# skmhrk1209/GANSynth

Measured on AMD Instinct MI355X. Metric: G+D step images/sec at 128x1024x2 mel+IF, higher is better.
Workload: dtype bf16; 1 GPU; BASELINE.json configs[1]: fully grown PGGAN 128x1024x2 G+D iteration (D update + G update, R1 + mode-seeking), per-GPU batch 8, random-init weights; global_batch=8, parallelism=dp1, launch=hipGraph replay, forked branches, forked_branches=True

## Files before the change

### gansynth_amd/_lib.py

```python
import ctypes
import os
from ctypes import c_char_p, c_double, c_float, c_int, c_int64, c_size_t, c_void_p, POINTER

_HERE = os.path.dirname(os.path.abspath(__file__))
LIB_PATH = os.path.join(_HERE, "libgansynth_hip.so")

GS_F32, GS_BF16 = 0, 1
ACT_NONE, ACT_LRELU, ACT_TANH = 0, 1, 2
ACT_LRELU_BITS, ACT_WRITE_BITS = 5, 16
PREP_CONV_FWD, PREP_CONV_BWD_DATA, PREP_CONVT_FWD, PREP_CONVT_BWD_DATA = 0, 1, 2, 3
CONV_FWD, CONV_BWD_DATA, CONV_BWD_WEIGHT = 0, 1, 2

P, I, F, L, Z = c_void_p, c_int, c_float, c_int64, c_size_t

SIGNATURES = {
    "gs_last_error": (c_char_p, []),
    "gs_version": (I, []),
    "gs_init": (I, []),
    "gs_streams_create": (I, [I, POINTER(P)]),
    "gs_streams_destroy": (I, [I, POINTER(P)]),
    "gs_prof_enable": (I, [I]),
    "gs_prof_collect": (I, [POINTER(c_int), POINTER(c_double), POINTER(c_double)]),
    "gs_prof_roofline": (I, [ctypes.c_double, ctypes.c_double, P, P, P]),
    "gs_prof_records": (I, [I, P, P, P, P, P]),
    "gs_comm_available": (I, []),
    "gs_comm_unique_id": (I, [P]),
    "gs_comm_init": (I, [POINTER(P), I, I, P]),
    "gs_comm_destroy": (I, [P]),
    "gs_comm_count": (I, [P, POINTER(I)]),
    "gs_allreduce_sum_f32": (I, [P, P, ctypes.c_int64, P]),
    "gs_comm_set_marker_us": (I, [P, ctypes.c_double]),
    "gs_broadcast_f32": (I, [P, P, ctypes.c_int64, I, P]),
    "gs_conv2d_workspace_bytes": (Z, [I, I, I, I, I, I, I, I, I]),
    "gs_conv2d_fwd": (I, [P, P, P, I, I, I, I, I, I, I, F, I, I, P, Z, P]),
    "gs_conv2d_fwd_bias_act": (I, [P, P, P, P, I, I, I, I, I, I, I, F, I, I, I, P, Z, P]),
    "gs_conv2d_bwd_data": (I, [P, P, P, I, I, I, I, I, I, I, F, I, I, P, Z, P]),
    "gs_conv2d_fwd_bias_act_norm": (I, [P, P, P, P, P, I, I, I, I, I, I, I, F, I, F, I, I, P, Z, P]),
    "gs_conv2d_transpose_s2_fwd_bias_act_norm": (I, [P, P, P, P, P, I, I, I, I, I, F, I, F, I, I, P, Z, P]),
    "gs_conv2d_fwd_mask": (I, [P, P, P, I, P, I, I, I, I, I, I, I, F, I, I, P, Z, P]),
    "gs_conv2d_bwd_data_mask": (I, [P, P, P, I, P, I, I, I, I, I, I, I, F, I, I, P, Z, P]),
    "gs_conv2d_bwd_weight": (I, [P, P, P, I, I, I, I, I, I, I, F, I, I, P, Z, P]),
    "gs_conv2d_bwd_weight_bias": (I, [P, P, P, P, I, I, I, I, I, I, I, F, I, I, P, Z, P]),
    "gs_conv2d_bwd_weight_bias_partial": (I, [P, P, P, P, I, I, I, I, I, I, I, F, I, I, P, Z, P, P]),
    "gs_conv2d_transpose_s2_bwd_weight_partial": (I, [P, P, P, I, I, I, I, I, F, I, I, P, Z, P, P]),
    "gs_wgrad_reduce_batch": (I, [P, I, P]),
    "gs_conv2d_bwd_weight_bias_multi": (I, [P, P, P, I, ctypes.c_uint, P, P, I, I, I, I, I, I, I, F, I, I, P, Z, P, P]),
    "gs_conv2d_transpose_s2_bwd_weight_multi": (I, [P, P, P, I, P, I, I, I, I, I, F, I, I, P, Z, P, P]),
    "gs_conv_wgrad_jobs_workspace_bytes": (Z, [P, I]),
    "gs_conv_wgrad_jobs": (I, [P, I, P, Z, P]),
    "gs_wgrad_cu_cap": (I, [I]),
    "gs_conv2d_transpose_s2_workspace_bytes": (Z, [I, I, I, I, I, I, I]),
    "gs_conv2d_transpose_s2_fwd": (I, [P, P, P, I, I, I, I, I, F, I, I, P, Z, P]),
    "gs_conv2d_transpose_s2_fwd_bias_act": (I, [P, P, P, P, I, I, I, I, I, F, I, I, I, P, Z, P]),
    "gs_conv2d_transpose_s2_bwd_data": (I, [P, P, P, I, I, I, I, I, F, I, I, P, Z, P]),
    "gs_conv2d_bwd_data_pnbwd_is_fused": (I, [I, I, I, I, I, I, I, I, I]),
    "gs_conv2d_fwd_pnbwdbwd_is_fused": (I, [I, I, I, I, I, I, I, I, I]),
    "gs_conv_igemm_config": (I, [I, I, I, I, I, I, I, I, POINTER(c_int)]),
    "gs_units_bias_act_to_nhwc": (I, [P, P, P, P, I, I, I, I, I, P]),
    "gs_nhwc_act_bwd_to_units": (I, [P, P, P, I, I, I, I, I, P]),
    "gs_conv2d_fwd_pnbwdbwd": (I, [P, P, P, P, I, F, P, P, I, I, I, I, I, I, I, F, I, I, P, Z, P]),
    "gs_conv2d_transpose_s2_fwd_pnbwdbwd": (I, [P, P, P, P, I, F, P, P, I, I, I, I, I, F, I, I, P, Z, P]),
    "gs_conv2d_bwd_data_pnbwd": (I, [P, P, P, P, I, F, P, I, I, I, I, I, I, I, F, I, I, P, Z, P]),
    "gs_conv2d_transpose_s2_bwd_data_pnbwd": (I, [P, P, P, P, I, F, P, I, I, I, I, I, F, I, I, P, Z, P]),
    "gs_conv2d_transpose_s2_bwd_weight": (I, [P, P, P, I, I, I, I, I, F, I, I, P, Z, P]),
    "gs_dense_fwd_workspace_bytes": (Z, [I, I, I]),
    "gs_dense_fwd": (I, [P, P, P, I, I, I, F, I, P, Z, P]),
    "gs_dense_fwd_bias_act": (I, [P, P, P, P, I, I, I, F, I, I, P, Z, P]),
    "gs_dense_fwd_bias_act_nhwc": (I, [P, P, P, P, I, I, I, I, F, I, I, P, Z, P]),
    "gs_dense_bwd_data": (I, [P, P, P, I, I, I, F, I, P]),
    "gs_dense_bwd_weight": (I, [P, P, P, I, I, I, F, I, I, P]),
    "gs_dense_fwd_nhwc": (I, [P, P, P, I, I, I, I, F, I, P, Z, P]),
    "gs_dense_bwd_data_nhwc": (I, [P, P, P, I, I, I, I, F, I, P]),
    "gs_dense_bwd_weight_nhwc": (I, [P, P, P, I, I, I, I, F, I, I, P]),
    "gs_embedding_fwd": (I, [P, P, P, I, I, I, F, I, P]),
    "gs_embedding_onehot_fwd": (I, [P, P, P, P, I, I, I, F, I, P]),
    "gs_embedding_bwd": (I, [P, P, P, I, I, I, F, I, P]),
    "gs_bias_act_fwd": (I, [P, P, P, L, I, I, I, P]),
    "gs_act_bwd": (I, [P, P, P, L, I, I, P]),
    "gs_act_bwd_bias": (I, [P, P, P, P, L, I, I, I, I, P, Z, P]),
    "gs_tanh_bwd_bwd": (I, [P, P, P, P, L, I, P]),
    "gs_channel_sum_workspace_bytes": (Z, [L, I]),
    "gs_channel_sum": (I, [P, P, L, I, I, I, P, Z, P]),
    "gs_bias_partial_rows": (I, [I, L, I, I]),
    "gs_channel_fold_batch_workspace_bytes": (Z, [P, I]),
    "gs_channel_fold_batch": (I, [P, I, P, Z, P]),
    "gs_pixel_norm_fwd": (I, [P, P, L, I, F, I, P]),
    "gs_pixel_norm_bwd": (I, [P, P, P, L, I, F, I, P]),
    "gs_pixel_norm_bwd_fused": (I, [P, P, P, P, L, I, F, I, I, I, P]),
    "gs_pixel_norm_bwd_bias_workspace_bytes": (Z, [L, I, I]),
    "gs_pixel_norm_bwd_fused_bias": (I, [P, P, P, P, P, L, I, F, I, I, I, I, P, Z, P]),
    "gs_pixel_norm_bwd_bwd_fused": (I, [P, P, P, P, P, L, I, F, I, I, P]),
# ... 92 lines not shown
```

### gansynth_amd/config.py

```python
import os

KNOBS = {
    "GS_TORCH_COLLECTIVES": ("operational", "gradient all-reduce through torch.distributed's communicator instead of the library's own (gs_comm_*)"),
    "GS_NO_GRAPH_ALLREDUCE": ("operational", "no RCCL collective inside captured graphs: eager all-reduce behind each replay (bench.DP_LADDER's tamer modes)"),
    "GS_FORK_PROBE": ("operational", "auto | always | never: probe a forked hipGraph replay in a child process before the first forked capture "
                                     "(auto: only on HIP builds the workaround was not debugged on, fork_probe._forked_replay_ok)"),
    "GS_FORK_PROBED": ("operational", "(set by the probe for child processes: ok | died)"),
    "GS_FORK_PROBE_TIMEOUT_S": ("operational", "budget of that probe, seconds (600)"),
    "GS_LEVEL_STREAMS": ("operational", "throw-away streams alive while a graph is instantiated (128; capture.Capture._leveled_queues)"),
    "GS_COMM_MARKER_US": ("operational", "tests / profiles at world size 1: the one-rank all-reduce becomes a kernel that holds its stream this long "
                                         "(read once per communicator, comm.RcclComm; gs_comm_set_marker_us)"),
    "GS_CAPTURE_MODE": ("operational", "debugging: force torch.cuda.graph's capture_error_mode"),
    "GS_DEBUG_POISON_WS": ("operational", "debugging: kernel workspaces start as NaN bit patterns"),
    "GS_CHECK_FUSION": ("operational", "debugging: every fused cross-node form also runs its unfused definition and the two are compared"),
    "GS_FORK_EAGER": ("operational", "tests: the forked branches with eager launches on two streams"),
    "GS_NO_FORK_MARKS": ("operational", "debugging: branches start where they are opened, not at their marks"),
    "GS_NO_FORK": ("schedule", "no parallel branches in the runs' graphs (5.9 against 5.2 ms; also taken when GPU_MAX_HW_QUEUES != 4 or the probe fails)"),
    "GS_NO_MERGED_RUNS": ("schedule", "part A of the generator run NOT inside the discriminator run's graph (5.13 against 4.99 ms)"),
    "GS_NO_FUSED_ITERATION": ("schedule", "two graphs per iteration with eager optimizer steps between them (neutral on one GPU; data parallel both "
                                          "all-reduces are then the last node of a graph)"),
    "GS_OVERLAP_REDUCE": ("schedule", "data parallel: round 4's four-graph iteration, each all-reduce on a forked branch beside part A of the other run "
                                      "(hides both collectives; +0.7 ms at world size 1)"),
    "GS_NO_OVERLAP_REDUCE": ("schedule", "(overrides GS_OVERLAP_REDUCE)"),
    "GS_DEBUG_DP_BUCKET": ("operational", "print the range the first message of a two-step discriminator all-reduce covers"),
    "GS_DP_BUCKET_D": ("schedule", "data parallel: the discriminator's gradient all-reduced in two steps, ~98 % of it beside the end of its backward (300-us stand-ins: -0.09 ... -0.14 ms fully grown, +0.15 in a fade-in)"),
    "GS_EARLY_FLUSH_DIV": ("schedule", "a layer is 'large' from 1/DIV of the full resolution's pixels (16)"),
    "GS_EARLY_FLUSH_CUS": ("schedule", "CUs the early weight-gradient contraction is sized for (192; 160 / 224 / 256 within noise, round 6)"),
    "GS_D_TAIL_LEVELS": ("schedule", "levels of the discriminator's tail run over [real; fake] as one batch when the runs do not fork (3)"),
    "GS_NO_EARLY_FLUSH": ("ablation", "weight gradients of the full-chip levels contracted at the end of the run only"),
    "GS_NO_DEFERRED_REDUCE": ("ablation", "every weight gradient contracted where autograd produces it"),
    "GS_NO_DEFERRED_FOLDS": ("ablation", "bias-gradient partial rows folded by their producers"),
    "GS_NO_WGRAD_GROUPS": ("ablation", "no grouped weight-gradient launches"),
    "GS_NO_SPLIT_G_LOSS": ("ablation", "the generator's loss as one launch over both halves: the mode-seeking second-order pass waits for the discriminator's forward"),
    "GS_NO_SPLIT_FINAL_FLUSH": ("ablation", "the final weight-gradient contraction of a run on one stream (HBM-bound and MFMA-bound jobs one after the other)"),
    "GS_NO_FUSED_LOSSES": ("ablation", "per-sample loss algebra in torch instead of the one-launch loss heads"),
    "GS_NO_D_TAIL_BATCH": ("ablation", "real and fake pass through the discriminator's tail separately (no-fork schedule)"),
    "GS_NO_FUSED_NORM": ("ablation", "pixel norm as its own node behind every generator conv"),
    "GS_NO_NORM_EPILOGUE": ("ablation", "no pixel norm in conv epilogues"),
    "GS_NO_NORM_BWD_EPILOGUE": ("ablation", "no previous-block norm backward in data-gradient epilogues"),
    "GS_NO_NORM_BWD2_EPILOGUE": ("ablation", "no second-order norm kernel in the forward-on-cotangent conv"),
    "GS_NO_NORM_BWD_BIAS": ("ablation", "bias sums outside the norm's backward"),
    "GS_NO_MASK_BITS": ("ablation", "leaky-relu masks read as the bf16 activations themselves, not as the sign bits stored behind them"),
    "GS_NO_PREMASK": ("ablation", "activation derivative never folded into the consuming data-gradient kernel"),
    "GS_NO_PREMASK_GRAPH": ("ablation", "... not across autograd nodes"),
    "GS_NO_PREMASK_GRAPH2": ("ablation", "... not in second-order graphs"),
    "GS_NO_PARAMS_ONLY": ("ablation", "leaf activations receive gradients like tf.gradients would not ask for"),
    "GS_NO_DERIVED_SLICES": ("ablation", "the 257-channel conv's weight slices copied on every use"),
    "GS_NO_UNITS_NHWC": ("ablation", "dense -> reshape -> activation as three steps"),
    "GS_NO_DENSE_NHWC": ("ablation", "flatten copy + plain dense kernels"),
}


def _check(name):
    if name not in KNOBS:
        raise KeyError("gansynth_amd.config: %s is not a registered environment switch (add it to KNOBS with its description)" % name)


def flag(name):
    _check(name)
    return bool(os.environ.get(name))


def value(name, default=None):
    _check(name)
    return os.environ.get(name, default)
```

### gansynth_amd/csrc/conv_api.hip

```cpp
#include "conv_shared.h"
#include <utility>
#include <vector>

namespace gs {


bool igemm_supported(int ic, int oc, int dtype);
bool igemm_norm_fused(int mode, int N, int Hb, int Wb, int IC, int OC, int dtype, int want);
int igemm_config(int mode, int N, int Hb, int Wb, int IC, int OC, int dtype, int want, int* out);
extern "C" int gs_pixel_norm_bwd_bwd_fused(const void* gg, const void* g, const void* x, void* out, void* out_g, int64_t p, int c, float eps, int pre_act,
                                           int dtype, void* stream);
bool wgrad_mfma_supported(int ic, int oc, int dtype);
size_t igemm_prep_bytes(int ic, int oc, int dtype);
int run_igemm(int mode, int variant, const void* x, const float* w_hwio, void* y, int N, int Hi, int Wi, int ICk,
              int OCk, int w_ci, int w_co, int Hb, int Wb, float alpha, const float* bias, int act, int dtype, int w_prepared,
              void* ws, size_t ws_bytes, hipStream_t st, const void* mask = nullptr, int mask_act = 0, void* y2 = nullptr, float pn_eps = 0.f,
              const void* addend = nullptr, int normbwd = 0);
extern "C" int gs_pixel_norm_bwd_fused(const void* g, const void* x, const void* addend, void* gx, int64_t p, int c, float eps, int pre_act, int post_act, int dtype,
                                       void* stream);
size_t wgrad_mfma_bytes(int mode, int dtype, int N, int Hb, int Wb, int IC, int OC);
bool wgrad_mfma_has_bias(int dtype);
int run_wgrad_mfma(int mode, const WgradSrcs& srcs, int nsrc, float* gw, float* gb, int N, int Hi, int Wi, int IC, int OC, int Hb,
                   int Wb, float alpha, int transpose, int accumulate, int dtype, void* ws, size_t ws_bytes, hipStream_t st,
                   GsWgradReduce* defer = nullptr);
bool wgrad_sk_supported(int mode, int dtype, int IC, int OC);
int wgrad_sk_tile_width(int Wb);
void wgrad_sk_job_geometry(int mode, int tw, int N, SkJob& q);
void wgrad_sk_plan(int mode, SkGroup& g);
size_t wgrad_sk_bytes(const SkGroup& g);
int run_wgrad_sk(int mode, int tw, const SkGroup& g, void* ws, size_t ws_bytes, hipStream_t st);

template <typename T, int OCV, int VEC>
__global__ void conv_direct_kernel(const T* __restrict__ x, const float* __restrict__ wp, T* __restrict__ y, int mode,
                                   int ks, int N, int Hi, int Wi, int IC, int OC, int Ho, int Wo, float alpha) {
    const int ngrp = OC / OCV;
    const long idx = (long)blockIdx.x * blockDim.x + threadIdx.x;
    const long total = (long)N * Ho * Wo * ngrp;
    if (idx >= total) return;
    const int g = idx % ngrp;
    long pix = idx / ngrp;
    const int ox = pix % Wo;
    pix /= Wo;
    const int oy = pix % Ho;
    const int n = pix / Ho;
    const int oc = g * OCV;
    float acc[OCV];
#pragma unroll
    for (int v = 0; v < OCV; ++v) acc[v] = 0.f;
    for (int ky = 0; ky < ks; ++ky) {
        int iy;
        if (mode == MODE_S1) iy = oy + ky - (ks >> 1);
        else if (mode == MODE_S2) iy = 2 * oy + ky;
        else { const int d = oy - ky; if (d < 0 || (d & 1)) continue; iy = d >> 1; }
        if (iy < 0 || iy >= Hi) continue;
        for (int kx = 0; kx < ks; ++kx) {
            int ix;
            if (mode == MODE_S1) ix = ox + kx - (ks >> 1);
            else if (mode == MODE_S2) ix = 2 * ox + kx;
            else { const int d = ox - kx; if (d < 0 || (d & 1)) continue; ix = d >> 1; }
            if (ix < 0 || ix >= Wi) continue;
            const T* xp = x + (((long)n * Hi + iy) * Wi + ix) * IC;
            const float* wr = wp + ((long)(ky * ks + kx) * OC + oc) * IC;
            if (VEC == 4) {
                for (int ic = 0; ic < IC; ic += 4) {
                    float xv[4];
                    ld4(xp + ic, xv);
#pragma unroll
                    for (int v = 0; v < OCV; ++v) {
                        const float4 wv = *reinterpret_cast<const float4*>(wr + (long)v * IC + ic);
                        acc[v] += xv[0] * wv.x + xv[1] * wv.y + xv[2] * wv.z + xv[3] * wv.w;
// ... 773 lines not shown
    if (int e = run_direct(mode, ksize, 0, x, w_hwio, z, n, h, w, ci, co, ci, co, hb, wb, alpha, dtype, w_prepared, ws, ws_bytes, st, bias, act, &fused, nullptr, 0, nullptr,
                           bits_out, &bits_done))
        return e;
    if (!fused && (bias || act != GS_ACT_NONE))
        if (int e = gs_bias_act_fwd(z, bias, z, (int64_t)n * hb * wb, co, act, dtype, stream)) return e;
    if (y2)
        if (int e = gs_pixel_norm_fwd(z, y2, (int64_t)n * hb * wb, co, pn_eps, dtype, stream)) return e;
    if (want_bits && !bits_done) return gs_pack_act_bits(y, (int64_t)n * hb * wb, co, dtype, stream);
    return 0;
}

extern "C" int gs_conv2d_fwd(const void* x, const float* w_hwio, void* y, int n, int h, int w, int ci, int co, int ksize,
                             int stride, float alpha, int dtype, int w_prepared, void* ws, size_t ws_bytes, void* stream) {
    return conv2d_fwd_impl(x, w_hwio, nullptr, GS_ACT_NONE, y, n, h, w, ci, co, ksize, stride, alpha, dtype, w_prepared, ws, ws_bytes, stream);
}

extern "C" int gs_conv2d_fwd_bias_act(const void* x, const float* w_hwio, const float* bias, void* y, int n, int h, int w, int ci, int co,
                                      int ksize, int stride, float alpha, int act, int dtype, int w_prepared, void* ws, size_t ws_bytes,
                                      void* stream) {
    return conv2d_fwd_impl(x, w_hwio, bias, act, y, n, h, w, ci, co, ksize, stride, alpha, dtype, w_prepared, ws, ws_bytes, stream);
}

extern "C" int gs_act_bwd(const void* g, const void* y, void* gx, int64_t numel, int act, int dtype, void* stream);

extern "C" int gs_conv2d_fwd_mask(const void* x, const float* w_hwio, const void* mask, int mask_act, void* y, int n, int h, int w, int ci, int co,
                                  int ksize, int stride, float alpha, int dtype, int w_prepared, void* ws, size_t ws_bytes, void* stream) {
    if (int e = check_conv_args(n, h, w, ci, co, ksize, stride, dtype)) return e;
    GS_CHECK_ARG(mask == nullptr || mask_act == GS_ACT_LRELU || mask_act == GS_ACT_TANH || mask_act == GS_ACT_LRELU_BITS, "conv2d_fwd_mask: bad activation %d", mask_act);
    hipStream_t st = as_stream(stream);
    const int hb = h / stride, wb = w / stride;
    const int mode = stride == 2 ? MODE_S2 : MODE_S1;
    const bool fused = mask != nullptr && co >= mask_fuse_min_channels() && ksize == 3 && igemm_supported(ci, co, dtype);
    int rc;
    const int bits_act = mask_act;
    if (mask_act == GS_ACT_LRELU_BITS) mask_act = GS_ACT_LRELU;
    if (ksize == 3 && igemm_supported(ci, co, dtype))
        rc = run_igemm(mode, 0, x, w_hwio, y, n, h, w, ci, co, ci, co, hb, wb, alpha, nullptr, GS_ACT_NONE, dtype, w_prepared, ws, ws_bytes, st, fused ? mask : nullptr, bits_act);
    else {
        bool epi = false, mdone = false;
        rc = run_direct(mode, ksize, 0, x, w_hwio, y, n, h, w, ci, co, ci, co, hb, wb, alpha, dtype, w_prepared, ws, ws_bytes, st, nullptr, GS_ACT_NONE, &epi, mask, mask_act, &mdone);
        if (rc || !mask || mdone) return rc;
    }
    if (rc || !mask || fused) return rc;
    return gs_act_bwd(y, mask, y, (int64_t)n * hb * wb * co, mask_act, dtype, stream);
}

extern "C" int gs_conv2d_fwd_bias_act_norm(const void* x, const float* w_hwio, const float* bias, void* z, void* y, int n, int h, int w, int ci, int co,
                                           int ksize, int stride, float alpha, int act, float eps, int dtype, int w_prepared, void* ws,
                                           size_t ws_bytes, void* stream) {
    GS_CHECK_ARG(y != nullptr, "conv2d_fwd_bias_act_norm: y is required (z is optional)");
    return conv2d_fwd_impl(x, w_hwio, bias, act, z, n, h, w, ci, co, ksize, stride, alpha, dtype, w_prepared, ws, ws_bytes, stream, y, eps);
}

extern "C" int gs_act_bwd(const void* g, const void* y, void* gx, int64_t numel, int act, int dtype, void* stream);

extern "C" int gs_conv2d_bwd_data_mask(const void* gy, const float* w_hwio, const void* mask, int mask_act, void* gx, int n, int h, int w, int ci, int co,
                                       int ksize, int stride, float alpha, int dtype, int w_prepared, void* ws, size_t ws_bytes, void* stream) {
    if (int e = check_conv_args(n, h, w, ci, co, ksize, stride, dtype)) return e;
    GS_CHECK_ARG(mask == nullptr || mask_act == GS_ACT_LRELU || mask_act == GS_ACT_TANH || mask_act == GS_ACT_LRELU_BITS, "conv2d_bwd_data_mask: bad activation %d", mask_act);
    const int bits_act = mask_act;
    if (mask_act == GS_ACT_LRELU_BITS) mask_act = GS_ACT_LRELU;
    const float* bias = nullptr;
    const int act = GS_ACT_NONE;
    hipStream_t st = as_stream(stream);
    const int hb = h / stride, wb = w / stride;
    int rc;
    bool fused = mask != nullptr && ci >= mask_fuse_min_channels();
    const void* km = fused ? mask : nullptr;
    if (stride == 1) {
        if (ksize == 3 && igemm_supported(co, ci, dtype))
            rc = run_igemm(MODE_S1, 1, gy, w_hwio, gx, n, h, w, co, ci, ci, co, h, w, alpha, bias, act, dtype, w_prepared, ws, ws_bytes, st, km, bits_act);
        else { rc = run_direct(MODE_S1, ksize, 1, gy, w_hwio, gx, n, h, w, co, ci, ci, co, h, w, alpha, dtype, w_prepared, ws, ws_bytes, st); fused = false; }
    } else if (igemm_supported(co, ci, dtype)) {
        rc = run_igemm(MODE_T2, 2, gy, w_hwio, gx, n, hb, wb, co, ci, ci, co, hb, wb, alpha, bias, act, dtype, w_prepared, ws, ws_bytes, st, km, bits_act);
    } else {
        rc = run_direct(MODE_T2, 3, 2, gy, w_hwio, gx, n, hb, wb, co, ci, ci, co, h, w, alpha, dtype, w_prepared, ws, ws_bytes, st);
        fused = false;
    }
    if (rc || !mask || fused) return rc;
    return gs_act_bwd(gx, mask, gx, (int64_t)n * h * w * ci, mask_act, dtype, stream);
}

extern "C" int gs_conv2d_bwd_data(const void* gy, const float* w_hwio, void* gx, int n, int h, int w, int ci, int co,
                                  int ksize, int stride, float alpha, int dtype, int w_prepared, void* ws, size_t ws_bytes, void* stream) {
    return gs_conv2d_bwd_data_mask(gy, w_hwio, nullptr, 0, gx, n, h, w, ci, co, ksize, stride, alpha, dtype, w_prepared, ws, ws_bytes, stream);
}

extern "C" size_t gs_channel_sum_workspace_bytes(int64_t p, int c);
extern "C" int gs_channel_sum(const void* g, float* out, int64_t p, int c, int accumulate, int dtype, void* ws, size_t ws_bytes, void* stream);

static WgradSrcs make_srcs(const void* const* xs, const void* const* gys, int nsrc, int n_per, const int* ns, unsigned bias_mask, bool swap, int* total) {
    WgradSrcs s;
    memset(&s, 0, sizeof(s));
    int end = 0;
    for (int i = 0; i < GS_WGRAD_MAX_SRC; ++i) {
        if (i < nsrc) {
            s.x[i] = swap ? gys[i] : xs[i];
            s.gy[i] = swap ? xs[i] : gys[i];
            end += ns ? ns[i] : n_per;
        }
        s.n_end[i] = end;
    }
    s.bias_mask = bias_mask;
    *total = end;
    return s;
}
// ... 197 lines not shown
                                                 jb.accumulate, jb.dtype, jws, jbytes, &d, stream);
        if (rc) return rc;
        if (jb.gw_ci_stride > jb.ci) {
            if (d.nslices <= 0 || d.transpose) return fail(GS_ERR_UNSUPPORTED, "conv_wgrad_jobs: a %d -> %d layer cannot add into a channel slice", jb.ci, jb.co);
            d.ic_ld = jb.gw_ci_stride;
        }
        if (d.nslices > 0) pend.push_back(d);
    }
    if (!pend.empty()) return gs_wgrad_reduce_batch(pend.data(), (int)pend.size(), stream);
    return 0;
}

extern "C" int gs_conv2d_bwd_weight(const void* x, const void* gy, float* gw_hwio, int n, int h, int w, int ci, int co,
                                    int ksize, int stride, float alpha, int accumulate, int dtype, void* ws, size_t ws_bytes, void* stream) {
    return gs_conv2d_bwd_weight_bias(x, gy, gw_hwio, nullptr, n, h, w, ci, co, ksize, stride, alpha, accumulate, dtype, ws, ws_bytes, stream);
}

extern "C" size_t gs_conv2d_transpose_s2_workspace_bytes(int which, int n, int h, int w, int ci, int co, int dtype) {
    if (which == GS_CONV_BWD_WEIGHT) {
        if (wgrad_mfma_supported(co, ci, dtype)) return wgrad_mfma_bytes(MODE_S2, dtype, n, h, w, co, ci);
        return wgrad_direct_bytes(3, n, h, w, co, ci);
    }
    return align256((size_t)9 * ci * co * 4);
}

static int conv2d_transpose_fwd_impl(const void* x, const float* w_hwio, const float* bias, int act, void* y, int n, int h, int w, int ci,
                                     int co, float alpha, int dtype, int w_prepared, void* ws, size_t ws_bytes, void* stream, void* y2 = nullptr,
                                     float pn_eps = 0.f) {
    if (int e = check_conv_args(n, 2 * h, 2 * w, co, ci, 3, 2, dtype)) return e;
    GS_CHECK_ARG(y || y2, "conv2d_transpose: no output");
    hipStream_t st = as_stream(stream);
    if (igemm_supported(ci, co, dtype) && act != GS_ACT_TANH)
        return run_igemm(MODE_T2, 0, x, w_hwio, y, n, h, w, ci, co, ci, co, h, w, alpha, bias, act, dtype, w_prepared, ws, ws_bytes, st, nullptr, 0, y2, pn_eps);
    void* z = y ? y : y2;
    if (int e = run_direct(MODE_T2, 3, 0, x, w_hwio, z, n, h, w, ci, co, ci, co, 2 * h, 2 * w, alpha, dtype, w_prepared, ws, ws_bytes, st)) return e;
    if (bias || act != GS_ACT_NONE)
        if (int e = gs_bias_act_fwd(z, bias, z, (int64_t)n * 4 * h * w, co, act, dtype, stream)) return e;
    if (y2) return gs_pixel_norm_fwd(z, y2, (int64_t)n * 4 * h * w, co, pn_eps, dtype, stream);
    return 0;
}

extern "C" int gs_conv2d_transpose_s2_fwd(const void* x, const float* w_hwio, void* y, int n, int h, int w, int ci, int co,
                                          float alpha, int dtype, int w_prepared, void* ws, size_t ws_bytes, void* stream) {
    return conv2d_transpose_fwd_impl(x, w_hwio, nullptr, GS_ACT_NONE, y, n, h, w, ci, co, alpha, dtype, w_prepared, ws, ws_bytes, stream);
}

extern "C" int gs_conv2d_transpose_s2_fwd_bias_act_norm(const void* x, const float* w_hwio, const float* bias, void* z, void* y, int n, int h, int w,
                                                        int ci, int co, float alpha, int act, float eps, int dtype, int w_prepared, void* ws,
                                                        size_t ws_bytes, void* stream) {
    GS_CHECK_ARG(y != nullptr, "conv2d_transpose_s2_fwd_bias_act_norm: y is required (z is optional)");
    return conv2d_transpose_fwd_impl(x, w_hwio, bias, act, z, n, h, w, ci, co, alpha, dtype, w_prepared, ws, ws_bytes, stream, y, eps);
}

extern "C" int gs_conv2d_transpose_s2_fwd_bias_act(const void* x, const float* w_hwio, const float* bias, void* y, int n, int h, int w, int ci,
                                                   int co, float alpha, int act, int dtype, int w_prepared, void* ws, size_t ws_bytes,
                                                   void* stream) {
    return conv2d_transpose_fwd_impl(x, w_hwio, bias, act, y, n, h, w, ci, co, alpha, dtype, w_prepared, ws, ws_bytes, stream);
}

extern "C" int gs_conv2d_transpose_s2_bwd_data(const void* gy, const float* w_hwio, void* gx, int n, int h, int w, int ci,
                                               int co, float alpha, int dtype, int w_prepared, void* ws, size_t ws_bytes, void* stream) {
    if (int e = check_conv_args(n, 2 * h, 2 * w, co, ci, 3, 2, dtype)) return e;
    const float* bias = nullptr;
    const int act = GS_ACT_NONE;
    hipStream_t st = as_stream(stream);
    if (igemm_supported(co, ci, dtype))
        return run_igemm(MODE_S2, 2, gy, w_hwio, gx, n, 2 * h, 2 * w, co, ci, ci, co, h, w, alpha, bias, act, dtype, w_prepared, ws, ws_bytes, st);
    return run_direct(MODE_S2, 3, 2, gy, w_hwio, gx, n, 2 * h, 2 * w, co, ci, ci, co, h, w, alpha, dtype, w_prepared, ws, ws_bytes, st);
}

extern "C" int gs_conv2d_fwd_pnbwdbwd(const void* x, const float* w_hwio, const void* g, const void* z, int act, float eps, void* out_g, void* out_z, int n, int h,
                                      int w, int ci, int co, int ksize, int stride, float alpha, int dtype, int w_prepared, void* ws, size_t ws_bytes, void* stream) {
    if (int e = check_conv_args(n, h, w, ci, co, ksize, stride, dtype)) return e;
    GS_CHECK_ARG(g && z && out_g && out_z && (act == GS_ACT_NONE || act == GS_ACT_LRELU), "conv2d_fwd_pnbwdbwd: g, z and both outputs are required, activation none or leaky relu (got %d)", act);
    hipStream_t st = as_stream(stream);
    const int hb = h / stride, wb = w / stride;
    if (ksize == 3 && igemm_supported(ci, co, dtype))
        return run_igemm(stride == 2 ? MODE_S2 : MODE_S1, 0, x, w_hwio, out_g, n, h, w, ci, co, ci, co, hb, wb, alpha, nullptr, GS_ACT_NONE, dtype, w_prepared, ws, ws_bytes, st,
                         z, act, out_z, eps, g, 2);
    if (int e = gs_conv2d_fwd(x, w_hwio, out_g, n, h, w, ci, co, ksize, stride, alpha, dtype, w_prepared, ws, ws_bytes, stream)) return e;
    return gs_pixel_norm_bwd_bwd_fused(out_g, g, z, out_z, out_g, (int64_t)n * hb * wb, co, eps, act, dtype, stream);
}
extern "C" int gs_conv2d_transpose_s2_fwd_pnbwdbwd(const void* x, const float* w_hwio, const void* g, const void* z, int act, float eps, void* out_g, void* out_z, int n,
                                                   int h, int w, int ci, int co, float alpha, int dtype, int w_prepared, void* ws, size_t ws_bytes, void* stream) {
    if (int e = check_conv_args(n, 2 * h, 2 * w, co, ci, 3, 2, dtype)) return e;
    GS_CHECK_ARG(g && z && out_g && out_z && (act == GS_ACT_NONE || act == GS_ACT_LRELU), "conv2d_transpose_s2_fwd_pnbwdbwd: g, z and both outputs are required, activation none or leaky relu (got %d)", act);
    hipStream_t st = as_stream(stream);
    if (igemm_supported(ci, co, dtype))
        return run_igemm(MODE_T2, 0, x, w_hwio, out_g, n, h, w, ci, co, ci, co, h, w, alpha, nullptr, GS_ACT_NONE, dtype, w_prepared, ws, ws_bytes, st, z, act, out_z, eps, g, 2);
    if (int e = gs_conv2d_transpose_s2_fwd(x, w_hwio, out_g, n, h, w, ci, co, alpha, dtype, w_prepared, ws, ws_bytes, stream)) return e;
    return gs_pixel_norm_bwd_bwd_fused(out_g, g, z, out_z, out_g, (int64_t)n * 4 * h * w, co, eps, act, dtype, stream);
}
extern "C" int gs_conv2d_fwd_pnbwdbwd_is_fused(int n, int h, int w, int ci, int co, int ksize, int stride, int transposed, int dtype) {
    if (ksize != 3 || !igemm_supported(ci, co, dtype)) return 0;
    if (transposed) return stride == 2 && igemm_norm_fused(MODE_T2, n, h, w, ci, co, dtype, IGEMM_NORM_BWD2) ? 1 : 0;
    return stride == 1 && igemm_norm_fused(MODE_S1, n, h, w, ci, co, dtype, IGEMM_NORM_BWD2) ? 1 : 0;
}

extern "C" int gs_conv2d_bwd_data_pnbwd(const void* gy, const float* w_hwio, const void* z, const void* addend, int act, float eps, void* gx, int n, int h, int w,
                                        int ci, int co, int ksize, int stride, float alpha, int dtype, int w_prepared, void* ws, size_t ws_bytes, void* stream) {
    if (int e = check_conv_args(n, h, w, ci, co, ksize, stride, dtype)) return e;
    GS_CHECK_ARG(z && gx && (act == GS_ACT_NONE || act == GS_ACT_LRELU), "conv2d_bwd_data_pnbwd: z is required, activation none or leaky relu (got %d)", act);
    hipStream_t st = as_stream(stream);
    if (stride == 1 && ksize == 3 && igemm_supported(co, ci, dtype))
        return run_igemm(MODE_S1, 1, gy, w_hwio, gx, n, h, w, co, ci, ci, co, h, w, alpha, nullptr, GS_ACT_NONE, dtype, w_prepared, ws, ws_bytes, st, z, act, nullptr, eps, addend, 1);
    if (stride == 1 && thin_expand_pnbwd_ok(ksize, co, ci, dtype)) {
// ... 64 lines not shown
```

### gansynth_amd/csrc/conv_igemm.hip

```cpp
#include <type_traits>
#include "conv_shared.h"
#include "gs_prof.h"

#ifndef GS_WGRAD_THIN_PREFETCH
#define GS_WGRAD_THIN_PREFETCH 1
#endif

extern "C" int gs_pixel_norm_fwd(const void* x, void* y, int64_t p, int c, float eps, int dtype, void* stream);
extern "C" int gs_pack_act_bits(void* z, int64_t p, int c, int dtype, void* stream);
extern "C" int gs_pixel_norm_bwd_fused(const void* g, const void* x, const void* addend, void* gx, int64_t p, int c, float eps, int pre_act, int post_act, int dtype,
                                       void* stream);
extern "C" int gs_pixel_norm_bwd_bwd_fused(const void* gg, const void* g, const void* x, void* out, void* out_g, int64_t p, int c, float eps, int pre_act,
                                           int dtype, void* stream);

namespace gs {

typedef float f32x16 __attribute__((ext_vector_type(16)));
typedef float f32x4 __attribute__((ext_vector_type(4)));
typedef __bf16 bf16x8 __attribute__((ext_vector_type(8)));


template <typename T> struct Mma;
template <> struct Mma<float> {
    typedef f32x4 frag_t;
    __device__ static inline void mma(const frag_t& a, const frag_t& b, f32x16& c) {
        c = __builtin_amdgcn_mfma_f32_32x32x2f32(a[0], b[0], c, 0, 0, 0);
        c = __builtin_amdgcn_mfma_f32_32x32x2f32(a[1], b[1], c, 0, 0, 0);
        c = __builtin_amdgcn_mfma_f32_32x32x2f32(a[2], b[2], c, 0, 0, 0);
        c = __builtin_amdgcn_mfma_f32_32x32x2f32(a[3], b[3], c, 0, 0, 0);
    }
};
template <> struct Mma<bf16_t> {
    typedef bf16x8 frag_t;
    __device__ static inline void mma(const frag_t& a, const frag_t& b, f32x16& c) {
        c = __builtin_amdgcn_mfma_f32_32x32x16_bf16(a, b, c, 0, 0, 0);
    }
};

template <int MODE> __host__ __device__ constexpr int patch_dim(int t) {
    return MODE == MODE_S1 ? t + 2 : (MODE == MODE_S2 ? 2 * t + 1 : t + 1);
}
template <int MODE> __host__ __device__ constexpr int tap_ky(int i) {
    return MODE == MODE_T2 ? (i < 4 ? (i >> 1) * 2 : (i < 6 ? (i - 4) * 2 : 1)) : i / 3;
}
template <int MODE> __host__ __device__ constexpr int tap_kx(int i) {
    return MODE == MODE_T2 ? (i < 4 ? (i & 1) * 2 : (i < 6 ? 1 : (i < 8 ? (i - 6) * 2 : 1))) : i % 3;
}
template <int MODE> __host__ __device__ constexpr int tap_phase(int i) {
    return MODE == MODE_T2 ? (i < 4 ? 0 : (i < 6 ? 1 : (i < 8 ? 2 : 3))) : 0;
}
template <int MODE> __host__ __device__ constexpr int tap_off(int k) {
    return MODE == MODE_T2 ? (k == 2 ? 0 : 1) : k;
}

struct ConvP {
    const void* x;
    const void* wp;
    void* y;
    const float* bias;
    int act;
    const void* mask;
    int mask_act;
    const unsigned char* mask_bits;
    unsigned char* bits_out;
    void* y2;
    float pn_eps;
    const void* addend;
    int normbwd;
    int* norm_pending;
    int N, Hi, Wi, IC, OC, Hb, Wb, tiles_x, tiles_y, nsp, noct, nch;
    unsigned m_noct, m_tx, m_ty;
    float alpha;
#ifdef GS_IGEMM_TRACE
    unsigned long long* trace;
#endif
};
#ifdef GS_IGEMM_TRACE
#define GS_TR(slot)                                                                                              \
    do {                                                                                                         \
        if (p.trace && threadIdx.x == 0 && (slot) < 64) {                                                        \
            p.trace[blockIdx.x * 64 + (slot)] = __builtin_amdgcn_s_memtime();                                    \
            if ((slot) == 0 || (slot) == 63) p.trace[4096 * 64 + blockIdx.x * 2 + ((slot) == 63)] = __builtin_amdgcn_s_memrealtime(); \
        }                                                                                                        \
    } while (0)
#else
#define GS_TR(slot) do { } while (0)
#endif

template <int N, int I = 0, typename F>
__device__ __forceinline__ void static_for(F&& f) {
    if constexpr (I < N) {
        f(std::integral_constant<int, I>{});
        static_for<N, I + 1>(f);
    }
}

typedef int i32x4 __attribute__((ext_vector_type(4)));

__device__ __forceinline__ void lds_dma16(unsigned lds_addr, unsigned voff, i32x4 rs) {
    asm volatile("s_mov_b32 m0, %0\n\ts_nop 0\n\tbuffer_load_dwordx4 %1, %2, 0 offen lds"
                 :
                 : "s"(lds_addr), "v"(voff), "s"(rs)
                 : "memory", "m0");
}
__device__ __forceinline__ void lds_dma16_s(unsigned lds_addr, unsigned voff, i32x4 rs, unsigned soff) {
    asm volatile("s_mov_b32 m0, %0\n\ts_nop 0\n\tbuffer_load_dwordx4 %1, %2, %3 offen lds"
                 :
                 : "s"(lds_addr), "v"(voff), "s"(rs), "s"(__builtin_amdgcn_readfirstlane(soff))
                 : "memory", "m0");
}
#ifndef GS_THIN_DMA_NT
#define GS_THIN_DMA_NT 0
#endif
__device__ __forceinline__ void lds_dma16_stream(unsigned lds_addr, unsigned voff, i32x4 rs) {
#if GS_THIN_DMA_NT
    asm volatile("s_mov_b32 m0, %0\n\ts_nop 0\n\tbuffer_load_dwordx4 %1, %2, 0 offen nt lds"
                 :
                 : "s"(lds_addr), "v"(voff), "s"(rs)
                 : "memory", "m0");
#else
    lds_dma16(lds_addr, voff, rs);
#endif
}
__device__ __forceinline__ i32x4 make_rsrc(const void* base, unsigned bytes) {
    const unsigned long long b = reinterpret_cast<unsigned long long>(base);
// ... 6 lines not shown
}
__device__ __forceinline__ void wait_vmcnt(int n) {
#define GS_VM(K) case K: asm volatile("s_waitcnt vmcnt(" #K ")" ::: "memory"); break;
    switch (n) {
        GS_VM(0) GS_VM(1) GS_VM(2) GS_VM(3) GS_VM(4) GS_VM(5) GS_VM(6) GS_VM(7) GS_VM(8) GS_VM(9) GS_VM(10) GS_VM(11)
        GS_VM(12) GS_VM(13) GS_VM(14) GS_VM(15) GS_VM(16) GS_VM(17) GS_VM(18) GS_VM(19) GS_VM(20) GS_VM(21) GS_VM(22)
        GS_VM(23) GS_VM(24) GS_VM(25) GS_VM(26) GS_VM(27) GS_VM(28) GS_VM(29) GS_VM(30) GS_VM(31) GS_VM(32)
        default: asm volatile("s_waitcnt vmcnt(0)" ::: "memory"); break;
    }
#undef GS_VM
}
__device__ __forceinline__ void block_barrier() {
    asm volatile("s_waitcnt lgkmcnt(0)" ::: "memory");
    __builtin_amdgcn_s_barrier();
    asm volatile("" ::: "memory");
}

#ifndef GS_NORM_EPI_PIPELINE
#define GS_NORM_EPI_PIPELINE 1
#endif
template <typename T, int MODE, int A, int B, int TW, int TG, bool RESIDENT, int D, int NORM, int RB = 64, bool SPEC = false, bool BITS = false>
__global__ __launch_bounds__(SPEC ? 512 : 256) void conv_igemm_kernel(const ConvP p) {
    static_assert(NORM >= 0 && NORM <= 3, "NORM: 0 plain, 1 pixel norm of the result (forward blocks), 2 pixel-norm backward of the result (data gradients), "
                                          "3 both gradients of a differentiated norm backward (second-order pass)");
    constexpr int NP = 128 * B;
    constexpr int TH = NP / TW;
    constexpr int PH = patch_dim<MODE>(TH), PW = patch_dim<MODE>(TW);
    constexpr int S = MODE == MODE_S2 ? 2 : 1;
    constexpr int NPH = MODE == MODE_T2 ? 4 : 1;
    constexpr int SZ = (int)sizeof(T);
    static_assert(RB == 64 || (RB == 128 && SZ == 2), "128-byte rows: bf16 only");
    constexpr int BK = RB / SZ;
    constexpr int SL = RB / 16;
    constexpr int KS = RB / 32;
    constexpr int OCT = 32 * A;
    constexpr int NTG = 9 / TG;
    constexpr int PCH = PH * PW * SL;
    constexpr int NPP = (PCH + 63) / 64;
    constexpr int PP = (NPP + 3) / 4;
    constexpr int PBUF = PP * 4096;
    constexpr int WBYTES = TG * OCT * RB;
    constexpr int NWP = WBYTES / 1024;
    constexpr int WP = (NWP + 3) / 4;
    constexpr int WBUF = WP * 4096;
    constexpr int NPB = 1 + (D + NTG - 1) / NTG;
    constexpr int NWB = D + 1;
    constexpr int NSTEP = KS * TG;
    typedef typename Mma<T>::frag_t frag_t;

    extern __shared__ __attribute__((aligned(16))) unsigned char lds[];
    unsigned char* const lpatch = lds;
    unsigned char* const lwgt = lds + NPB * PBUF;
    float* const lbias = reinterpret_cast<float*>(lwgt + (RESIDENT ? p.nch : NWB) * WBUF);
    const unsigned a_patch = (unsigned)(uintptr_t)lds;
    const unsigned a_wgt = a_patch + NPB * PBUF;

    const T* __restrict__ wp = reinterpret_cast<const T*>(p.wp);
    T* __restrict__ y = reinterpret_cast<T*>(p.y);
    const int Hi = p.Hi, Wi = p.Wi, IC = p.IC, OC = p.OC, Hb = p.Hb, Wb = p.Wb, NCH = p.nch;

    const int tid = threadIdx.x;
    const int lane = tid & 63, hi = lane >> 5, l31 = lane & 31;
    const int wv8 = __builtin_amdgcn_readfirstlane(tid >> 6);
    const bool loader = SPEC && wv8 >= 4;
    const bool issuer = !SPEC || loader;
    const bool computer = !SPEC || !loader;
    const int wv = wv8 & 3;

    const int total = p.nsp * p.noct;
    int first, stride, count;
    if ((gridDim.x & 7) == 0) {
        const int per_xcd = (total + 7) >> 3, gx = gridDim.x >> 3;
        const int xcd = blockIdx.x & 7, loc = blockIdx.x >> 3;
        first = xcd * per_xcd + loc;
        stride = gx;
        int end = (xcd + 1) * per_xcd;
        if (end > total) end = total;
        count = first < end ? (end - first + gx - 1) / gx : 0;
    } else {
        first = blockIdx.x;
        stride = gridDim.x;
        count = first < total ? (total - first + stride - 1) / stride : 0;
    }
    if (count == 0) return;
    GS_TR(0);

    int p_voff[PP], p_lx[PP];
#pragma unroll
    for (int k = 0; k < PP; ++k) {
        const int slot = (wv + 4 * k) * 64 + lane;
        const int row = slot / SL, pos = slot % SL;
        const int ly = row / PW, lx = row - ly * PW;
        p_voff[k] = ((ly * Wi + lx) * IC) * SZ + ((pos ^ (RB == 64 ? (lx >> 2) & 3 : (lx >> 1) & 7)) << 4);
        p_lx[k] = slot < PCH ? lx : 0x40000000;
    }
    constexpr int RPP = 1024 / RB;
    constexpr int SUBS = OCT / RPP;
    const int w_lane0 = RB == 64 ? ((lane >> 2) * IC) * SZ + (((lane & 3) ^ ((lane >> 4) & 3)) << 4)
                                 : ((lane >> 3) * IC) * SZ + (((lane & 7) ^ (lane >> 4)) << 4);
    const int w_lane1 = RB == 64 ? w_lane0 : ((lane >> 3) * IC) * SZ + (((lane & 7) ^ (4 + (lane >> 4))) << 4);
    int w_soff[NTG][WP];
    bool w_odd[WP];
#pragma unroll
    for (int k = 0; k < WP; ++k) w_odd[k] = RB == 128 && (((wv + 4 * k) % SUBS) & 1);
#pragma unroll
    for (int tg = 0; tg < NTG; ++tg)
// ... 65 lines not shown
                --i_left;
                i_item += stride;
                if (i_left > 0) item_coords(i_item, i_n, i_by, i_bx, i_oc0);
                else i_left = 0;
            }
        }
    };

    f32x16 acc[NPH][A][B];
    auto zero_acc = [&]() __attribute__((always_inline)) {
#pragma unroll
        for (int ph = 0; ph < NPH; ++ph)
#pragma unroll
            for (int a = 0; a < A; ++a)
#pragma unroll
                for (int b = 0; b < B; ++b)
#pragma unroll
                    for (int r = 0; r < 16; ++r) acc[ph][a][b][r] = 0.f;
    };

    int b_off[B][3][KS], a_off[KS];
#pragma unroll
    for (int b = 0; b < B; ++b) {
        const int q = (wv * B + b) * 32 + l31;
        const int pb0 = ((q / TW) * S) * PW + (q % TW) * S;
#pragma unroll
        for (int ox = 0; ox < 3; ++ox) {
            const int lx = (q % TW) * S + ox;
            const int key = RB == 64 ? (lx >> 2) & 3 : (lx >> 1) & 7;
#pragma unroll
            for (int ks = 0; ks < KS; ++ks) b_off[b][ox][ks] = (pb0 + ox) * RB + (((ks * 2 + hi) ^ key) << 4);
        }
    }
#pragma unroll
    for (int ks = 0; ks < KS; ++ks) a_off[ks] = l31 * RB + (((ks * 2 + hi) ^ (RB == 64 ? (l31 >> 2) & 3 : (l31 >> 1) & 7)) << 4);

    GS_TR(1);
    if (issuer) {
        if (RESIDENT) {
            for (int ch = 0; ch < NCH; ++ch)
#pragma unroll
                for (int k = 0; k < WP; ++k) issue_weight_piece(k, 0, (i_oc0 * IC + ch * BK) * SZ, a_wgt + ch * WBUF);
        }
#pragma unroll
        for (int d = 0; d < D; ++d) {
            issue_setup(d % NTG);
#pragma unroll
            for (int q = 0; q < stage_pieces(d % NTG); ++q) issue_piece(q, d % NTG);
            issue_advance(d % NTG);
        }
    }
    GS_TR(2);
    for (int c = tid; c < OC; c += (SPEC ? 512 : 256)) lbias[c] = p.bias ? p.bias[c] : 0.f;
    zero_acc();
    if (computer) {
#pragma unroll
        for (int b = 0; b < B; ++b)
#pragma unroll
            for (int ox = 0; ox < 3; ++ox)
#pragma unroll
                for (int ks = 0; ks < KS; ++ks) asm volatile("" : "+v"(b_off[b][ox][ks]));
#pragma unroll
        for (int ks = 0; ks < KS; ++ks) asm volatile("" : "+v"(a_off[ks]));
#pragma unroll
        for (int ph = 0; ph < NPH; ++ph)
#pragma unroll
            for (int a = 0; a < A; ++a)
#pragma unroll
                for (int b = 0; b < B; ++b) asm volatile("" : "+v"(acc[ph][a][b]));
    }
    wait_vmcnt(0);
    block_barrier();
    GS_TR(3);
#ifdef GS_IGEMM_TRACE
    int tr_stage = 0;
#endif

    int item = first, done = 0, c_pb = 0, c_wb = 0;
    while (true) {
        int n, by, bx, oc0;
        item_coords(item, n, by, bx, oc0);
        unsigned mbw[BITS ? B * (MODE == MODE_T2 ? 4 : 1) : 1][A];
        constexpr bool NPIPE = (NORM == 2 || NORM == 3) && A * B <= 2 && GS_NORM_EPI_PIPELINE;
        typedef typename std::conditional<SZ == 4, float4, uint4>::type nvec_t;
        constexpr int NNV = SZ == 4 ? 4 : 2;
        nvec_t nz[NPIPE ? 2 : 1][A][NNV], nx[NPIPE ? 2 : 1][A][NNV];
        auto norm_fetch = [&](int i, nvec_t (&zq)[A][NNV], nvec_t (&xq)[A][NNV]) __attribute__((always_inline)) {
            constexpr int NPHB = MODE == MODE_T2 ? 4 : 1;
            const int b = i / NPHB, ph = i % NPHB;
            const int Ho = MODE == MODE_T2 ? 2 * Hb : Hb, Wo = MODE == MODE_T2 ? 2 * Wb : Wb;
            const int q = (wv * B + b) * 32 + l31;
            const int gy = by + q / TW, gx = bx + q % TW;
            const int oy = MODE == MODE_T2 ? 2 * gy + (ph >> 1) : gy;
            const int ox = MODE == MODE_T2 ? 2 * gx + (ph & 1) : gx;
            const long base = (gy < Hb && gx < Wb) ? (((long)n * Ho + oy) * Wo + ox) * OC + oc0 : 0;
#ifdef GS_ABL_NOMASKLOAD
            const long zbase = base & 1023;
#else
            const long zbase = base;
#endif
#pragma unroll
            for (int a = 0; a < A; ++a)
#pragma unroll
                for (int v = 0; v < NNV; ++v) {
                    zq[a][v] = *reinterpret_cast<const nvec_t*>(reinterpret_cast<const T*>(p.mask) + zbase + a * 32 + v * (32 / NNV) + hi * (16 / NNV));
                    if (NORM == 3 || p.addend)
// ... 369 lines not shown
                                        }
                                }
                                ssq = swap32_sum(ssq); shg = swap32_sum(shg);
                                shz = swap32_sum(shz); szg = swap32_sum(szg);
                                const float inv_c = 1.f / (float)(32 * A);
                                const float r = rsqrtf(ssq * inv_c + p.pn_eps);
                                const float r2 = r * r, r3 = r2 * r;
                                const float ma = shg * inv_c, mb = shz * inv_c, mm = szg * inv_c;
                                const float kz = 3.f * r3 * r2 * mb * mm - r3 * ma;
#pragma unroll
                                for (int a = 0; a < A; ++a)
#pragma unroll
                                    for (int v = 0; v < NV; ++v) {
                                        float o1[EV], o2[EV];
#pragma unroll
                                        for (int e = 0; e < EV; ++e) {
                                            const float zc = zv[a][v][e], gc = gv[a][v][e], hc = hv[a][v][e];
                                            o1[e] = r * (hc - zc * r2 * mb);
                                            o2[e] = kz * zc - r3 * (mm * hc + mb * gc);
                                        }
                                        if (inside) {
                                            if constexpr (SZ == 4) {
                                                st4(reinterpret_cast<float*>(y) + off + a * 32 + v * 8 + hi * 4, o1);
                                                st4(reinterpret_cast<float*>(p.y2) + off + a * 32 + v * 8 + hi * 4, o2);
                                            } else {
                                                uint4 w4;
                                                w4.x = pack_bf16x2(o1[0], o1[1]); w4.y = pack_bf16x2(o1[2], o1[3]); w4.z = pack_bf16x2(o1[4], o1[5]); w4.w = pack_bf16x2(o1[6], o1[7]);
                                                *reinterpret_cast<uint4*>(reinterpret_cast<bf16_t*>(y) + off + a * 32 + v * 16 + hi * 8) = w4;
                                                w4.x = pack_bf16x2(o2[0], o2[1]); w4.y = pack_bf16x2(o2[2], o2[3]); w4.z = pack_bf16x2(o2[4], o2[5]); w4.w = pack_bf16x2(o2[6], o2[7]);
                                                *reinterpret_cast<uint4*>(reinterpret_cast<bf16_t*>(p.y2) + off + a * 32 + v * 16 + hi * 8) = w4;
                                            }
                                        }
                                    }
                            } else if constexpr (NORM == 1) {
                                float o[A][4][4], ssq = 0.f;
#pragma unroll
                                for (int a = 0; a < A; ++a) {
                                    finish(ph, a, b, o[a]);
#pragma unroll
                                    for (int k = 0; k < 16; ++k) ssq += o[a][k >> 2][k & 3] * o[a][k >> 2][k & 3];
                                }
                                ssq = swap32_sum(ssq);
                                const float r = rsqrtf(ssq * (1.f / (float)(32 * A)) + p.pn_eps);
#pragma unroll
                                for (int a = 0; a < A; ++a) {
                                    if (y) {
                                        float oz[4][4];
#pragma unroll
                                        for (int k = 0; k < 16; ++k) oz[k >> 2][k & 3] = o[a][k >> 2][k & 3];
                                        store(y, off, a, oz, inside, static_cast<const mvec_t*>(nullptr));
                                    }
#pragma unroll
                                    for (int k = 0; k < 16; ++k) o[a][k >> 2][k & 3] *= r;
                                    store(reinterpret_cast<T*>(p.y2), off, a, o[a], inside, static_cast<const mvec_t*>(nullptr));
                                }
                            } else {
                                mvec_t mz_one[A][NV];
                                if constexpr (!MASK_ALL) {
                                    if (p.mask) mask_fetch(off, inside, mz_one);
                                }
#pragma unroll
                                for (int a = 0; a < A; ++a) {
                                    float o[4][4];
                                    finish(ph, a, b, o);
                                    const mvec_t* mz = MASK_ALL ? mz_all[MASK_ALL ? b * NPH + ph : 0][a] : mz_one[a];
                                    store(y, off, a, o, inside, mz, p.mask ? (use_mb ? 2 : 1) : 0, emit_bits);
                                }
                            }
                        }
                    }
                    zero_acc();
                }
#endif
                block_barrier();
#ifdef GS_IGEMM_TRACE
                GS_TR(4 + tr_stage);
                ++tr_stage;
#endif
                if (tg == NTG - 1) c_pb = c_pb + 1 == NPB ? 0 : c_pb + 1;
                if (!RESIDENT) c_wb = c_wb + 1 == NWB ? 0 : c_wb + 1;
            }
        }
        if (++done >= count) break;
        item += stride;
    }
    GS_TR(63);
    wait_vmcnt(0);
}

template <typename T, int MODE, int TW>
__global__ __launch_bounds__(256) void conv_wgrad_kernel(
    const WgradSrcs srcs, float* __restrict__ part,
    int N, int Hi, int Wi, int IC, int OC, int Hb, int Wb, int tiles_x, int tiles_y, int ntiles, int nslices) {
    constexpr int NP = MODE == MODE_S2 ? 64 : 128;
    constexpr int TH = NP / TW;
    constexpr int PH = patch_dim<MODE>(TH), PW = patch_dim<MODE>(TW);
    constexpr int S = MODE == MODE_S2 ? 2 : 1;
    constexpr int ROWF = 32;
    constexpr int LDS_MAIN = (PH * PW + NP) * ROWF;
    constexpr int LDS_RED = 4 * 1024;
    __shared__ __attribute__((aligned(16))) float lds[LDS_MAIN > LDS_RED ? LDS_MAIN : LDS_RED];
    float* lp = lds;
    float* lg = lds + PH * PW * ROWF;

    const int tid = threadIdx.x;
    const int lane = tid & 63, wv = tid >> 6, hi = lane >> 5, l31 = lane & 31;
    const int n_ict = IC / 32;
// ... 920 lines not shown
static int g_wgrad_cu_cap = 0;
static int wgrad_cus() {
    const int n = num_cus();
    return g_wgrad_cu_cap > 0 && g_wgrad_cu_cap < n ? g_wgrad_cu_cap : n;
}

#ifndef GS_MAX_BLOCKS_PER_CU
#define GS_MAX_BLOCKS_PER_CU 2
#endif
#ifndef GS_SMALL_D
#define GS_SMALL_D 2
#endif
template <typename T, int MODE, int A, int B, int TW, int TG, bool RESIDENT = false, int D = 2, int NORM = 0, int RB = 64, bool SPEC = false, bool BITS = false>
static int launch_igemm(ConvP p, hipStream_t st) {
    if constexpr (!BITS && sizeof(T) == 2 && NORM == 0) {
        if (p.mask_bits || p.bits_out) return launch_igemm<T, MODE, A, B, TW, TG, RESIDENT, D, NORM, RB, SPEC, true>(p, st);
    }
    constexpr int NP = 128 * B;
    constexpr int TH = NP / TW;
    constexpr int PH = patch_dim<MODE>(TH), PW = patch_dim<MODE>(TW);
    constexpr int OCT = 32 * A;
    constexpr int BK = RB / (int)sizeof(T);
    constexpr int NTG = 9 / TG;
    constexpr int PBUF = ((PH * PW * (RB / 16) + 255) / 256) * 4096;
    constexpr int WBUF = ((TG * OCT * RB + 4095) / 4096) * 4096;
    constexpr int NPB = 1 + (D + NTG - 1) / NTG, NWB = D + 1;
    p.tiles_x = cdiv(p.Wb, TW);
    p.tiles_y = cdiv(p.Hb, TH);
    p.nsp = p.N * p.tiles_x * p.tiles_y;
    p.noct = cdiv(p.OC, OCT);
    p.nch = p.IC / BK;
    {
        auto magic = [](int d) { return d <= 1 ? 0u : (unsigned)(((1ull << 32) + (unsigned)d - 1) / (unsigned)d); };
        if (p.noct >= 2048 || p.tiles_x >= 2048 || p.tiles_y >= 2048)
            return fail(GS_ERR_UNSUPPORTED, "conv igemm: %d channel tiles / %d x %d spatial tiles exceed the item decoder's range", p.noct, p.tiles_x, p.tiles_y);
        static const long max_items = getenv("GS_IGEMM_MAX_ITEMS") ? atol(getenv("GS_IGEMM_MAX_ITEMS")) : (1L << 21);
        if ((long)p.nsp * p.noct >= max_items) {
            const long per_image = (long)p.tiles_x * p.tiles_y * p.noct;
            const int chunk = (int)((max_items - 1) / per_image);
            if (chunk < 1) return fail(GS_ERR_UNSUPPORTED, "conv igemm: %ld work items per image exceed the item decoder's range", per_image);
            const size_t in_img = (size_t)p.Hi * p.Wi * p.IC * sizeof(T);
            const size_t out_img = (size_t)p.Hb * p.Wb * (MODE == MODE_T2 ? 4 : 1) * p.OC * sizeof(T);
            auto adv = [](const void* q, size_t b) -> const void* { return q ? (const char*)q + b : nullptr; };
            for (int n0 = 0; n0 < p.N; n0 += chunk) {
                ConvP q = p;
                q.N = p.N - n0 < chunk ? p.N - n0 : chunk;
                q.x = adv(p.x, n0 * in_img);
                q.y = const_cast<void*>(adv(p.y, n0 * out_img));
                q.y2 = const_cast<void*>(adv(p.y2, n0 * out_img));
                q.mask = adv(p.mask, n0 * out_img);
                q.mask_bits = reinterpret_cast<const unsigned char*>(adv(p.mask_bits, n0 * out_img / (8 * sizeof(T))));
                q.bits_out = reinterpret_cast<unsigned char*>(const_cast<void*>(adv(p.bits_out, n0 * out_img / (8 * sizeof(T)))));
                q.addend = adv(p.addend, n0 * out_img);
                int pending = 0;
                if (p.norm_pending) q.norm_pending = &pending;
                if (int e = launch_igemm<T, MODE, A, B, TW, TG, RESIDENT, D, NORM, RB, SPEC, BITS>(q, st)) return e;
                if (p.norm_pending && pending) *p.norm_pending = pending;
            }
            return 0;
        }
        p.m_noct = magic(p.noct); p.m_tx = magic(p.tiles_x); p.m_ty = magic(p.tiles_y);
    }
    const int wbufs = RESIDENT ? p.nch : NWB;
    const size_t lds = (size_t)NPB * PBUF + (size_t)wbufs * WBUF + (size_t)((p.OC + 3) / 4) * 16 + 0;
    if (p.OC % OCT != 0) return fail(GS_ERR_UNSUPPORTED, "conv igemm: %d output channels with %d-wide tiles", p.OC, OCT);
    if ((size_t)p.Hi * p.Wi * p.IC * sizeof(T) >= (1ull << 31)) return fail(GS_ERR_UNSUPPORTED, "conv igemm: one image exceeds 2 GiB");
    if (lds > 160 * 1024) return fail(GS_ERR_UNSUPPORTED, "conv igemm: %zu bytes of LDS needed", lds);
    if (NORM && p.OC != OCT) return fail(GS_ERR_UNSUPPORTED, "conv igemm: fused pixel norm needs the whole channel range in one tile");
    if ((NORM == 2 || NORM == 3) && p.OC != OCT) return fail(GS_ERR_UNSUPPORTED, "conv igemm: fused pixel-norm backward needs the whole channel range in one tile");
    if (!((NORM == 2 && p.normbwd == 1) || (NORM == 3 && p.normbwd == 2)) && p.normbwd) {
        if (p.norm_pending) *p.norm_pending = 1 + p.normbwd;
        p.normbwd = 0;
        p.mask = nullptr;
        p.addend = nullptr;
        p.y2 = nullptr;
    }
    if (NORM != 1 && NORM != 3 && p.y2) {
        if (!p.y) p.y = p.y2;
        p.y2 = nullptr;
        if (p.norm_pending) *p.norm_pending = 1;
    }
    if (p.IC % BK != 0) return fail(GS_ERR_UNSUPPORTED, "conv igemm: %d input channels with %d-channel chunks", p.IC, BK);
    auto kern = conv_igemm_kernel<T, MODE, A, B, TW, TG, RESIDENT, D, NORM, RB, SPEC, BITS>;
    static size_t max_set = 0;
    if (lds > max_set) {
        if (hipFuncSetAttribute(reinterpret_cast<const void*>(kern), hipFuncAttributeMaxDynamicSharedMemorySize, (int)lds) != hipSuccess)
            return fail(GS_ERR_HIP, "conv igemm: cannot reserve %zu bytes of dynamic LDS", lds);
        max_set = lds;
    }
    int per_cu = (int)((160 * 1024) / lds);
    if (per_cu > GS_MAX_BLOCKS_PER_CU) per_cu = GS_MAX_BLOCKS_PER_CU;
    if (per_cu < 1 || SPEC) per_cu = 1;
    const long total = (long)p.nsp * p.noct;
    long grid = (long)per_cu * num_cus();
    if (grid > total) grid = total;
    if (grid >= 8) grid &= ~7L;
    const double flops = 2.0 * 9.0 * (double)p.N * p.Hb * p.Wb * p.IC * p.OC;
    const double out_px = (double)p.N * p.Hb * p.Wb * (MODE == MODE_T2 ? 4 : 1);
    const double bytes = ((double)p.N * p.Hi * p.Wi * p.IC + out_px * p.OC * (1.0 + (p.mask ? (p.mask_bits ? 1.0 / 16.0 : 1.0) : 0.0) + (p.bits_out ? 1.0 / 16.0 : 0.0) + ((NORM == 1 && p.y) ? 1.0 : 0.0) + ((NORM == 2 && p.addend) ? 1.0 : 0.0) + (NORM == 3 ? 2.0 : 0.0)) + 9.0 * p.IC * p.OC) * sizeof(T);
    const int reps = prof_reps();
    ProfScope ps(st, flops, bytes, MODE, p.N, p.Hb, p.Wb, p.IC, p.OC, p.mask ? 1 : 0, NORM ? 1 : 0, reps);
    for (int r = 0; r < reps; ++r) hipLaunchKernelGGL(kern, dim3((unsigned)grid), dim3(SPEC ? 512 : 256), lds, st, p);
    return 0;
}

struct IgemmCfg {
    int A, B, TW, TG;
    bool RESIDENT = false;
    int D = 2, NORM = IGEMM_PLAIN, RB = 64;
    bool SPEC = false;
    bool operator==(const IgemmCfg& o) const {
        return A == o.A && B == o.B && TW == o.TW && TG == o.TG && RESIDENT == o.RESIDENT && D == o.D && NORM == o.NORM && RB == o.RB && SPEC == o.SPEC;
    }
};
struct IgemmKnobs { bool no_small_tiles, no_rb128, spec; };
static IgemmKnobs igemm_knobs() {
    static const IgemmKnobs k = {getenv("GS_NO_SMALL_TILES") != nullptr, getenv("GS_NO_RB128") != nullptr,
                                 getenv("GS_SPEC") ? (atoi(getenv("GS_SPEC")) & 1) != 0 : true};
    return k;
}

static IgemmCfg choose_igemm(int mode, int dtype, int N, int Hb, int Wb, int IC, int OC, int want, long cus, IgemmKnobs knobs) {
    constexpr int FWD = 1 << IGEMM_NORM_FWD, BWD = 1 << IGEMM_NORM_BWD, BWD2 = 1 << IGEMM_NORM_BWD2;
    auto epi = [&](int forms) { return (forms >> want) & 1 ? want : IGEMM_PLAIN; };
    const int nch = IC / (dtype == GS_F32 ? 16 : 32);
    const bool a2 = OC % 64 == 0;
    const int tw = Wb >= 32 ? 32 : 16;
    auto items64 = [&](int B_) { return (long)N * cdiv(Hb, 4 * B_) * cdiv(Wb, 32) * (OC / 64); };
    const bool small = !knobs.no_small_tiles && items64(1) <= cus;
    const bool rb128 = dtype == GS_BF16 && !knobs.no_rb128 && IC % 64 == 0;
    if (mode == MODE_S2) {
        if (small) return {1, 1, tw, 9, false, 1};
        if (!a2) return {1, 1, 32, 3};
        if (OC == 64 && nch == 1 && Wb >= 32 && items64(1) >= cus) return {2, 1, 32, 9, true, 1, epi(BWD)};
        if (OC % 128 == 0 && Wb >= 32 && (long)N * cdiv(Hb, 4) * cdiv(Wb, 32) * (OC / 128) >= cus) return {4, 1, 32, 3};
        return {2, 1, tw, 3};
    }
    const bool s1 = mode == MODE_S1;
    if (OC == 32 && nch <= 2 && Wb >= 64) return {1, s1 ? 2 : 1, 64, 9, true, 1, epi(s1 ? FWD | BWD | BWD2 : FWD | BWD2)};
    if (small) {
        if (rb128) return {1, 1, tw, 9, false, 1, IGEMM_PLAIN, 128, knobs.spec};
        return {1, 1, tw, 9, false, GS_SMALL_D};
    }
    if (!a2) return {1, 1, s1 ? 32 : tw, 3};
    if (!s1) return {2, 1, tw, 3, false, 2, Wb >= 32 && OC == 64 ? epi(FWD | BWD2) : IGEMM_PLAIN};
    if (Wb >= 32 && items64(2) >= 2 * cus) return {2, 2, 32, 3, false, 1, OC == 64 ? epi(FWD | BWD | BWD2) : IGEMM_PLAIN};
    if (OC == 64 && nch <= 2 && Wb >= 32 && items64(2) >= cus / 2) return {2, 2, 32, 9, true};
    if (Wb >= 32 && items64(2) >= cus) {
        if (rb128) return {2, 2, 32, 3, false, 1, IGEMM_PLAIN, 128};
        return {2, 2, 32, 3};
    }
    return {2, 1, tw, 3};
// ... 11 lines not shown
    X(MODE_S1, false, 1, 2, 64, 9, true, 1, IGEMM_NORM_BWD, 64, false)          \
    X(MODE_S1, false, 1, 2, 64, 9, true, 1, IGEMM_NORM_BWD2, 64, false)         \
    X(MODE_S1, true, 1, 1, 32, 9, false, 1, IGEMM_PLAIN, 128, true)             \
    X(MODE_S1, true, 1, 1, 16, 9, false, 1, IGEMM_PLAIN, 128, true)             \
    X(MODE_S1, true, 1, 1, 32, 9, false, 1, IGEMM_PLAIN, 128, false)            \
    X(MODE_S1, true, 1, 1, 16, 9, false, 1, IGEMM_PLAIN, 128, false)            \
    X(MODE_S1, false, 1, 1, 32, 9, false, GS_SMALL_D, IGEMM_PLAIN, 64, false)   \
    X(MODE_S1, false, 1, 1, 16, 9, false, GS_SMALL_D, IGEMM_PLAIN, 64, false)   \
    X(MODE_S1, false, 1, 1, 32, 3, false, 2, IGEMM_PLAIN, 64, false)            \
    X(MODE_S1, false, 2, 2, 32, 3, false, 1, IGEMM_PLAIN, 64, false)            \
    X(MODE_S1, false, 2, 2, 32, 3, false, 1, IGEMM_NORM_FWD, 64, false)         \
    X(MODE_S1, false, 2, 2, 32, 3, false, 1, IGEMM_NORM_BWD, 64, false)         \
    X(MODE_S1, false, 2, 2, 32, 3, false, 1, IGEMM_NORM_BWD2, 64, false)        \
    X(MODE_S1, false, 2, 2, 32, 9, true, 2, IGEMM_PLAIN, 64, false)             \
    X(MODE_S1, true, 2, 2, 32, 3, false, 1, IGEMM_PLAIN, 128, false)            \
    X(MODE_S1, false, 2, 2, 32, 3, false, 2, IGEMM_PLAIN, 64, false)            \
    X(MODE_S1, false, 2, 1, 32, 3, false, 2, IGEMM_PLAIN, 64, false)            \
    X(MODE_S1, false, 2, 1, 16, 3, false, 2, IGEMM_PLAIN, 64, false)            \
    X(MODE_S2, false, 1, 1, 32, 9, false, 1, IGEMM_PLAIN, 64, false)            \
    X(MODE_S2, false, 1, 1, 16, 9, false, 1, IGEMM_PLAIN, 64, false)            \
    X(MODE_S2, false, 1, 1, 32, 3, false, 2, IGEMM_PLAIN, 64, false)            \
    X(MODE_S2, false, 2, 1, 32, 9, true, 1, IGEMM_PLAIN, 64, false)             \
    X(MODE_S2, false, 2, 1, 32, 9, true, 1, IGEMM_NORM_BWD, 64, false)          \
    X(MODE_S2, false, 4, 1, 32, 3, false, 2, IGEMM_PLAIN, 64, false)            \
    X(MODE_S2, false, 2, 1, 32, 3, false, 2, IGEMM_PLAIN, 64, false)            \
    X(MODE_S2, false, 2, 1, 16, 3, false, 2, IGEMM_PLAIN, 64, false)            \
    X(MODE_T2, false, 1, 1, 64, 9, true, 1, IGEMM_PLAIN, 64, false)             \
    X(MODE_T2, false, 1, 1, 64, 9, true, 1, IGEMM_NORM_FWD, 64, false)          \
    X(MODE_T2, false, 1, 1, 64, 9, true, 1, IGEMM_NORM_BWD2, 64, false)         \
    X(MODE_T2, true, 1, 1, 32, 9, false, 1, IGEMM_PLAIN, 128, true)             \
    X(MODE_T2, true, 1, 1, 16, 9, false, 1, IGEMM_PLAIN, 128, true)             \
    X(MODE_T2, true, 1, 1, 32, 9, false, 1, IGEMM_PLAIN, 128, false)            \
    X(MODE_T2, true, 1, 1, 16, 9, false, 1, IGEMM_PLAIN, 128, false)            \
    X(MODE_T2, false, 1, 1, 32, 9, false, GS_SMALL_D, IGEMM_PLAIN, 64, false)   \
    X(MODE_T2, false, 1, 1, 16, 9, false, GS_SMALL_D, IGEMM_PLAIN, 64, false)   \
    X(MODE_T2, false, 1, 1, 32, 3, false, 2, IGEMM_PLAIN, 64, false)            \
    X(MODE_T2, false, 1, 1, 16, 3, false, 2, IGEMM_PLAIN, 64, false)            \
    X(MODE_T2, false, 2, 1, 32, 3, false, 2, IGEMM_PLAIN, 64, false)            \
    X(MODE_T2, false, 2, 1, 32, 3, false, 2, IGEMM_NORM_FWD, 64, false)         \
    X(MODE_T2, false, 2, 1, 32, 3, false, 2, IGEMM_NORM_BWD2, 64, false)        \
    X(MODE_T2, false, 2, 1, 16, 3, false, 2, IGEMM_PLAIN, 64, false)            \
    GS_IGEMM_FORCED(X)

static bool igemm_instantiated(int mode, int dtype, const IgemmCfg& c) {
#define GS_ROW(M, BF16_ONLY, ...) if (mode == M && (dtype == GS_BF16 || !BF16_ONLY) && c == IgemmCfg{__VA_ARGS__}) return true;
    GS_IGEMM_CONFIGS(GS_ROW)
#undef GS_ROW
    return false;
}

template <typename T, int MODE>
static int dispatch_igemm(ConvP p, hipStream_t st) {
    constexpr int dtype = sizeof(T) == 4 ? GS_F32 : GS_BF16;
    const int want = p.normbwd ? 1 + p.normbwd : (p.y2 ? IGEMM_NORM_FWD : IGEMM_PLAIN);
    IgemmCfg c = choose_igemm(MODE, dtype, p.N, p.Hb, p.Wb, p.IC, p.OC, want, num_cus(), igemm_knobs());
#ifdef GS_FORCE_CFG
    if (MODE == GS_FORCE_MODE && dtype == GS_BF16) c = IgemmCfg{GS_FORCE_CFG};
#endif
#define GS_ROW(M, BF16_ONLY, A, B, TW, TG, RESIDENT, D, NORM, RB, SPEC)                                \
    if constexpr (MODE == M && (dtype == GS_BF16 || !BF16_ONLY))                                       \
        if (c == IgemmCfg{A, B, TW, TG, RESIDENT, D, NORM, RB, SPEC}) return launch_igemm<T, MODE, A, B, TW, TG, RESIDENT, D, NORM, RB, SPEC>(p, st);
    GS_IGEMM_CONFIGS(GS_ROW)
#undef GS_ROW
    return fail(GS_ERR_UNSUPPORTED, "conv igemm: no instantiation of mode %d dtype %d A=%d B=%d TW=%d TG=%d RESIDENT=%d D=%d NORM=%d RB=%d SPEC=%d", MODE, dtype,
                c.A, c.B, c.TW, c.TG, (int)c.RESIDENT, c.D, c.NORM, c.RB, (int)c.SPEC);
}

bool igemm_supported(int ic, int oc, int dtype) {
    const int bk = dtype == GS_F32 ? 16 : 32;
    return ic % bk == 0 && oc % 32 == 0;
}
bool igemm_norm_fused(int mode, int N, int Hb, int Wb, int IC, int OC, int dtype, int want) {
    return igemm_supported(IC, OC, dtype) && choose_igemm(mode, dtype, N, Hb, Wb, IC, OC, want, num_cus(), igemm_knobs()).NORM == want;
}
int igemm_config(int mode, int N, int Hb, int Wb, int IC, int OC, int dtype, int want, int* out) {
    if (mode < MODE_S1 || mode > MODE_T2 || (dtype != GS_F32 && dtype != GS_BF16) || want < IGEMM_PLAIN || want > IGEMM_NORM_BWD2 || N < 1 || Hb < 1 || Wb < 1 || !out)
        return fail(GS_ERR_ARG, "conv igemm config: bad mode %d / dtype %d / epilogue %d / shape %d x %d x %d", mode, dtype, want, N, Hb, Wb);
    if (!igemm_supported(IC, OC, dtype)) return fail(GS_ERR_UNSUPPORTED, "conv igemm config: %d -> %d channels do not run on the implicit GEMM", IC, OC);
    const IgemmCfg c = choose_igemm(mode, dtype, N, Hb, Wb, IC, OC, want, num_cus(), igemm_knobs());
    const int v[10] = {c.A, c.B, c.TW, c.TG, c.RESIDENT, c.D, c.NORM, c.RB, c.SPEC, igemm_instantiated(mode, dtype, c)};
    memcpy(out, v, sizeof(v));
    return 0;
}
bool wgrad_mfma_supported(int ic, int oc, int dtype) { return (dtype == GS_F32 || dtype == GS_BF16) && ic % 32 == 0 && oc % 32 == 0; }

size_t igemm_prep_bytes(int ic, int oc, int dtype) {
    return align256((size_t)9 * ic * oc * (dtype == GS_F32 ? 4 : 2));
}

template <typename T>
static int run_igemm_t(int mode, int variant, const void* x, const float* w_hwio, void* y, int N, int Hi, int Wi,
                       int ICk, int OCk, int w_ci, int w_co, int Hb, int Wb, float alpha, const float* bias, int act,
                       int w_prepared, void* ws, size_t ws_bytes, hipStream_t st, const void* mask, int mask_act, void* y2, float pn_eps,
                       const void* addend, int normbwd) {
    const size_t need = (size_t)9 * w_ci * w_co * sizeof(T);
    if (ws_bytes < need) return fail(GS_ERR_WORKSPACE, "conv igemm: workspace %zu < %zu", ws_bytes, need);
    T* wp = reinterpret_cast<T*>(ws);
    const long total = 9L * w_ci * w_co;
    if (!w_prepared)
        hipLaunchKernelGGL((weight_prep_kernel<T>), dim3(cdiv(total, 256)), dim3(256), 0, st, w_hwio, wp, 9, w_ci, w_co, variant);
    ConvP p;
    memset(&p, 0, sizeof(p));
    const size_t out_numel = (size_t)N * Hb * Wb * (mode == MODE_T2 ? 4 : 1) * OCk;
    const bool plain = y2 == nullptr && !normbwd;
    const bool write_bits = (act & GS_ACT_WRITE_BITS) != 0;
    act &= ~GS_ACT_WRITE_BITS;
    if (mask_act == GS_ACT_LRELU_BITS) {
        mask_act = GS_ACT_LRELU;
        if (sizeof(T) == 2 && plain && mask && OCk % 32 == 0) p.mask_bits = reinterpret_cast<const unsigned char*>(mask) + out_numel * sizeof(T);
    }
    bool bits_pending = write_bits;
    if (write_bits && sizeof(T) == 2 && plain && y && act == GS_ACT_LRELU && OCk % 32 == 0 && (!mask || p.mask_bits)) {
        p.bits_out = reinterpret_cast<unsigned char*>(y) + out_numel * sizeof(T);
        bits_pending = false;
    }
    p.x = x; p.wp = wp; p.y = y; p.bias = bias; p.act = act; p.mask = mask; p.mask_act = mask_act;
    p.N = N; p.Hi = Hi; p.Wi = Wi; p.IC = ICk; p.OC = OCk; p.Hb = Hb; p.Wb = Wb; p.alpha = alpha;
    int pending = 0;
    p.y2 = y2; p.pn_eps = pn_eps; p.norm_pending = &pending;
    p.addend = normbwd ? addend : nullptr; p.normbwd = normbwd;
    int rc;
    if (mode == MODE_S1) rc = dispatch_igemm<T, MODE_S1>(p, st);
    else if (mode == MODE_S2) rc = dispatch_igemm<T, MODE_S2>(p, st);
    else rc = dispatch_igemm<T, MODE_T2>(p, st);
    if (rc) return rc;
    GS_CHECK_LAUNCH();
    if (pending == 3) {
        const long px = (long)N * Hb * Wb * (mode == MODE_T2 ? 4 : 1);
        return gs_pixel_norm_bwd_bwd_fused(y, addend, mask, y2, y, px, OCk, pn_eps, mask_act, sizeof(T) == 4 ? GS_F32 : GS_BF16, st);
    }
    if (pending == 2) {
        const long px = (long)N * Hb * Wb * (mode == MODE_T2 ? 4 : 1);
        return gs_pixel_norm_bwd_fused(y, mask, addend, y, px, OCk, pn_eps, GS_ACT_NONE, mask_act, sizeof(T) == 4 ? GS_F32 : GS_BF16, st);
    }
    if (pending) {
        const long px = (long)N * Hb * Wb * (mode == MODE_T2 ? 4 : 1);
        if (int e = gs_pixel_norm_fwd(y ? y : y2, y2, px, OCk, pn_eps, sizeof(T) == 4 ? GS_F32 : GS_BF16, st)) return e;
    }
    if (bits_pending && y)
        return gs_pack_act_bits(y, (int64_t)(out_numel / OCk), OCk, sizeof(T) == 4 ? GS_F32 : GS_BF16, st);
    return 0;
}

int run_igemm(int mode, int variant, const void* x, const float* w_hwio, void* y, int N, int Hi, int Wi, int ICk,
              int OCk, int w_ci, int w_co, int Hb, int Wb, float alpha, const float* bias, int act, int dtype, int w_prepared,
              void* ws, size_t ws_bytes, hipStream_t st, const void* mask, int mask_act, void* y2, float pn_eps, const void* addend, int normbwd) {
    GS_DISPATCH_DTYPE(dtype, return (run_igemm_t<T>(mode, variant, x, w_hwio, y, N, Hi, Wi, ICk, OCk, w_ci, w_co, Hb,
                                                    Wb, alpha, bias, act, w_prepared, ws, ws_bytes, st, mask, mask_act, y2, pn_eps, addend, normbwd)));
}

static int patch_dim_rt(int mode, int t) { return mode == MODE_S1 ? t + 2 : (mode == MODE_S2 ? 2 * t + 1 : t + 1); }
static bool wgrad_2x2(int mode, int dtype, int IC, int OC) { (void)mode; return dtype == GS_BF16 && IC % 64 == 0 && OC % 64 == 0; }
static bool wgrad_thin_pairs(int mode, int dtype, int IC, int OC) {
    static const bool off = getenv("GS_NO_THIN_PAIRS") != nullptr;
    return !off && dtype == GS_BF16 && !wgrad_2x2(mode, dtype, IC, OC) && OC % 64 == 0;
}
static bool wgrad_thin_dma(int mode, int dtype, int IC, int OC, int Wb) {
    static const bool off = getenv("GS_NO_THIN_DMA") != nullptr;
    (void)mode;
    return !off && dtype == GS_BF16 && IC == 32 && (OC == 32 || OC == 64) && Wb >= 32;
}
static void wgrad_geometry(int mode, int dtype, int N, int Hb, int Wb, int IC, int OC, int* tw, int* tiles_x, int* tiles_y,
                           int* ntiles, int* nslices) {
    int np = (mode == MODE_S2 ? 64 : 128) * (dtype == GS_BF16 ? 2 : 1);
    if (mode == MODE_S2 && wgrad_2x2(mode, dtype, IC, OC)) np = 64;
    if (wgrad_thin_dma(mode, dtype, IC, OC, Wb)) {
        np = mode == MODE_S2 ? 64 : 256;
        *tw = 32;
        const int th = np / 32;
        *tiles_x = cdiv(Wb, 32);
        *tiles_y = cdiv(Hb, th);
        *ntiles = N * *tiles_x * *tiles_y;
        const int lds = 2 * (((patch_dim_rt(mode, th) * patch_dim_rt(mode, 32) + 15) / 16) * 1024 + (OC / 32) * np * 64);
        int per_cu = (160 * 1024) / lds;
        if (per_cu > 2) per_cu = 2;
        if (per_cu < 1) per_cu = 1;
        int ns = per_cu * wgrad_cus();
        if (ns > *ntiles) ns = *ntiles;
        *nslices = ns;
        return;
    }
    *tw = Wb >= 32 ? 32 : 16;
    const int th = np / *tw;
    *tiles_x = cdiv(Wb, *tw);
    *tiles_y = cdiv(Hb, th);
    *ntiles = N * *tiles_x * *tiles_y;
    int pairs = (IC / 32) * (OC / 32);
    int target = dtype == GS_BF16 ? 768 : 512;
    if (wgrad_2x2(mode, dtype, IC, OC)) { pairs /= 4; target = 256; }
    else if (wgrad_thin_pairs(mode, dtype, IC, OC)) pairs /= 2;
    int ns = target / pairs;
    if (ns < 1) ns = 1;
    if (ns > *ntiles) ns = *ntiles;
    *nslices = ns;
}

bool wgrad_mfma_has_bias(int dtype) { return dtype == GS_BF16; }
size_t wgrad_mfma_bytes(int mode, int dtype, int N, int Hb, int Wb, int IC, int OC) {
    int tw, tx, ty, nt, ns;
    wgrad_geometry(mode, dtype, N, Hb, Wb, IC, OC, &tw, &tx, &ty, &nt, &ns);
    return align256((size_t)ns * (9 * (size_t)IC * OC + OC) * sizeof(float));
// ... 234 lines not shown
```

### gansynth_amd/csrc/conv_shared.h

```cpp
#pragma once
#include "gs_common.h"

namespace gs {

enum { MODE_S1 = 0, MODE_S2 = 1, MODE_T2 = 2 };
enum { IGEMM_PLAIN = 0, IGEMM_NORM_FWD = 1, IGEMM_NORM_BWD = 2, IGEMM_NORM_BWD2 = 3 };
#define GS_WGRAD_MAX_SRC 4

static inline size_t align256(size_t v) { return (v + 255) & ~(size_t)255; }

struct WgradSrcs {
    const void* x[GS_WGRAD_MAX_SRC];
    const void* gy[GS_WGRAD_MAX_SRC];
    int n_end[GS_WGRAD_MAX_SRC];
    unsigned bias_mask;
};
__device__ __forceinline__ int wgrad_source(const WgradSrcs& s, int nn, int& n_local) {
    const int src = (nn >= s.n_end[0]) + (nn >= s.n_end[1]) + (nn >= s.n_end[2]);
    n_local = nn - (src ? s.n_end[src - 1] : 0);
    return src;
}

#define GS_SK_MAX_JOBS 16
#define GS_SK_PSTRIDE (9 * 64 * 64 + 64)
struct SkJob {
    WgradSrcs srcs;
    float* gw;
    float* gb;
    float alpha;
    int transpose, accumulate;
    int Hi, Wi, IC, OC, Hb, Wb;
    int ICld;
    int tiles_x, tiles_y, ntiles;
    int n_ict, nct;
    int unit_base, run_base;
};
struct SkGroup {
    int njobs, total_units, total_runs, nblocks;
    SkJob job[GS_SK_MAX_JOBS];
};
__host__ __device__ inline int sk_block_of(long u, long nb, long total) { return (int)(((u + 1) * nb - 1) / total); }

template <typename T>
__global__ void weight_prep_kernel(const float* __restrict__ w, T* __restrict__ wp, int taps, int ci, int co, int variant) {
    long idx = (long)blockIdx.x * blockDim.x + threadIdx.x;
    long total = (long)taps * ci * co;
    if (idx >= total) return;
    if (variant == 0) {
        int c_i = idx % ci;
        int c_o = (idx / ci) % co;
        int t = idx / ((long)ci * co);
        DT<T>::st(wp + idx, w[((long)t * ci + c_i) * co + c_o]);
    } else {
        int t = idx / ((long)ci * co);
        long rem = idx % ((long)ci * co);
        int tt = variant == 1 ? taps - 1 - t : t;
        DT<T>::st(wp + (long)tt * ci * co + rem, w[idx]);
    }
}
// ... 187 lines not shown
```

### gansynth_amd/functional.py

```python
import contextlib
import itertools

import torch
from torch.autograd.function import once_differentiable

_NODE_SEQ = itertools.count(1 << 40)


def _number_node(out):
    t = out[0] if isinstance(out, (tuple, list)) and out else out
    fn = getattr(t, "grad_fn", None) if isinstance(t, torch.Tensor) else None
    if fn is not None and hasattr(fn, "_set_sequence_nr"):
        fn._set_sequence_nr(next(_NODE_SEQ))


class Function(torch.autograd.Function):

    @classmethod
    def apply(cls, *args, **kwargs):
        out = super().apply(*args, **kwargs)
        _number_node(out)
        return out


# ... 35 lines not shown


class tap_pair(object):

    def __init__(self, a, b):
        self.pair = None if a is None or b is None else (a, b)

    def __enter__(self):
        if activation_tap.active is not None:
            activation_tap.active.pair = self.pair
        return self

    def __exit__(self, *exc):
        if activation_tap.active is not None:
            activation_tap.active.pair = None
        return False


def _tap(z, act):
    tap = activation_tap.active
    if tap is not None and act == ACT_LRELU:
        if tap.pair is not None:
            n = z.shape[0] // 2
            tap.calls[tap.pair[0]][1].append(z[:n].detach())
            tap.calls[tap.pair[1]][1].append(z[n:].detach())
        else:
            tap.calls[-1][1].append(z.detach())


class _ConvKind(object):

    def __init__(self, ksize, stride):
        self.ksize, self.stride = ksize, stride

    def fwd(self, x, w, alpha):
        return _K().conv2d_fwd(x, w, self.ksize, self.stride, alpha)

    def fwd_bias_act(self, x, w, bias, alpha, act):
        return _K().conv2d_fwd_bias_act(x, w, bias, self.ksize, self.stride, alpha, act)

    def fwd_mask(self, x, w, alpha, mask, mask_act):
        K = _K()
        if hasattr(K, "conv2d_fwd_mask"):
            return K.conv2d_fwd_mask(x, w, self.ksize, self.stride, alpha, mask, mask_act)
        return K.act_bwd(self.fwd(x, w, alpha), mask, mask_act)

    def fwd_bias_act_norm(self, x, w, bias, alpha, act, eps, want_z):
        K = _K()
        if hasattr(K, "conv2d_fwd_bias_act_norm"):
            return K.conv2d_fwd_bias_act_norm(x, w, bias, self.ksize, self.stride, alpha, act, eps, want_z=want_z)
        z = self.fwd_bias_act(x, w, bias, alpha, act)
        return z, K.pixel_norm_fwd(z, eps)

    def bwd_data(self, gy, w, x_shape, alpha):
        return _K().conv2d_bwd_data(gy, w, x_shape, self.ksize, self.stride, alpha)

    def bwd_data_mask(self, gy, w, x_shape, alpha, mask, mask_act):
        return _K().conv2d_bwd_data(gy, w, x_shape, self.ksize, self.stride, alpha, mask=mask, mask_act=mask_act)

    def bwd_data_pnbwd(self, gy, w, x_shape, alpha, z, eps, act, addend):
        return _K().conv2d_bwd_data_pnbwd(gy, w, x_shape, self.ksize, self.stride, alpha, z, eps, act, addend=addend)

    def bwd_data_pnbwd_is_fused(self, x_shape, co, dtype):
        K = _K()
        return hasattr(K, "bwd_data_pnbwd_is_fused") and K.bwd_data_pnbwd_is_fused(x_shape, co, self.ksize, self.stride, False, dtype)

    def fwd_pnbwdbwd(self, x, w, alpha, g, z, eps, act):
        return _K().conv2d_fwd_pnbwdbwd(x, w, self.ksize, self.stride, alpha, g, z, eps, act)

    def fwd_pnbwdbwd_is_fused(self, x_shape, co, dtype):
        K = _K()
        return hasattr(K, "fwd_pnbwdbwd_is_fused") and K.fwd_pnbwdbwd_is_fused(x_shape, co, self.ksize, self.stride, False, dtype)

    bias_in_wgrad = True

    def bwd_weight(self, x, gy, alpha, out=None, bias_out=None):
        return _K().conv2d_bwd_weight(x, gy, self.ksize, self.stride, alpha, out=out, bias_out=bias_out)


class _ConvTransposeKind(object):

    def fwd(self, x, w, alpha):
        return _K().conv2d_transpose_fwd(x, w, alpha)

    def fwd_bias_act(self, x, w, bias, alpha, act):
        return _K().conv2d_transpose_fwd_bias_act(x, w, bias, alpha, act)

    def fwd_bias_act_norm(self, x, w, bias, alpha, act, eps, want_z):
        K = _K()
        if hasattr(K, "conv2d_transpose_fwd_bias_act_norm"):
            return K.conv2d_transpose_fwd_bias_act_norm(x, w, bias, alpha, act, eps, want_z=want_z)
        z = self.fwd_bias_act(x, w, bias, alpha, act)
        return z, K.pixel_norm_fwd(z, eps)

    def bwd_data(self, gy, w, x_shape, alpha):
        return _K().conv2d_transpose_bwd_data(gy, w, alpha)

    def bwd_data_pnbwd(self, gy, w, x_shape, alpha, z, eps, act, addend):
        return _K().conv2d_transpose_bwd_data_pnbwd(gy, w, alpha, z, eps, act, addend=addend)

    def bwd_data_pnbwd_is_fused(self, x_shape, co, dtype):
        K = _K()
        return hasattr(K, "bwd_data_pnbwd_is_fused") and K.bwd_data_pnbwd_is_fused(x_shape, co, 3, 2, True, dtype)

    def fwd_pnbwdbwd(self, x, w, alpha, g, z, eps, act):
        return _K().conv2d_transpose_fwd_pnbwdbwd(x, w, alpha, g, z, eps, act)

    def fwd_pnbwdbwd_is_fused(self, x_shape, co, dtype):
        K = _K()
        return hasattr(K, "fwd_pnbwdbwd_is_fused") and K.fwd_pnbwdbwd_is_fused(x_shape, co, 3, 2, True, dtype)

    def bwd_weight(self, x, gy, alpha, out=None):
        return _K().conv2d_transpose_bwd_weight(x, gy, alpha, out=out)


class _DenseKind(object):

    def fwd(self, x, w, alpha):
        return _K().dense_fwd(x, w, alpha)

    def fwd_bias_act(self, x, w, bias, alpha, act):
        if hasattr(_K(), "dense_fwd_bias_act"):
            return _K().dense_fwd_bias_act(x, w, bias, alpha, act)
        return _K().bias_act_fwd(_K().dense_fwd(x, w, alpha), bias, act)

    def bwd_data(self, gy, w, x_shape, alpha):
        return _K().dense_bwd_data(gy, w, alpha)

    def bwd_weight(self, x, gy, alpha, out=None):
        return _K().dense_bwd_weight(x, gy, alpha, out=out)


class _DenseFlatKind(object):

    def fwd(self, x, w, alpha):
        return _K().dense_fwd_nhwc(x, w, alpha)

    def fwd_bias_act(self, x, w, bias, alpha, act):
        if hasattr(_K(), "dense_fwd_bias_act"):
            return _K().dense_fwd_bias_act(x, w, bias, alpha, act)
        return _K().bias_act_fwd(_K().dense_fwd_nhwc(x, w, alpha), bias, act)

    def bwd_data(self, gy, w, x_shape, alpha):
        return _K().dense_bwd_data_nhwc(gy, w, x_shape, alpha)

    def bwd_weight(self, x, gy, alpha, out=None):
# ... 220 lines not shown
        if up is not None and ctx.needs_input_grad[0] and not torch.is_grad_enabled():
            g_gy = ctx.kind.fwd_mask(t, w, ctx.alpha, up.saved_tensors[2], up.act)
            if _CHECK_FUSION:
                _check_fused("fwd_mask", g_gy, _K().act_bwd(ctx.kind.fwd(t, w, ctx.alpha), up.saved_tensors[2], up.act))
            up._gs_gg_premasked = g_gy.data_ptr()
        else:
            g_gy = _Bilinear.apply(t, w, ctx.kind, ctx.alpha) if ctx.needs_input_grad[0] else None
        g_w = None
        if ctx.needs_input_grad[1]:
            tgt = _accum_target(ctx.wref)
            if tgt is None:
                tgt = _slice_target(ctx.wref, t, gy, ctx.kind)
            if tgt is not None:
                ctx.kind.bwd_weight(t, gy, ctx.alpha, out=tgt)
            else:
                g_w = _BilinearBwdWeight.apply(t, gy, ctx.kind, ctx.alpha).to(w.dtype)
        return g_gy, g_w, None, None, None, None


class _BilinearBwdWeight(Function):

    @staticmethod
    def forward(ctx, x, gy, kind, alpha):
        ctx.kind, ctx.alpha = kind, alpha
        ctx.save_for_backward(x, gy)
        return kind.bwd_weight(x, gy, alpha)

    @staticmethod
    def backward(ctx, ggw):
        x, gy = ctx.saved_tensors
        g_x = _BilinearBwdData.apply(gy, ggw, x.shape, ctx.kind, ctx.alpha) if ctx.needs_input_grad[0] else None
        g_gy = _Bilinear.apply(x, ggw, ctx.kind, ctx.alpha) if ctx.needs_input_grad[1] else None
        return g_x, g_gy, None, None


def _bias_act_backward(gz, z, act, bias_param, want_b):
    plain = not torch.is_grad_enabled()
    tgt = _accum_target(bias_param) if want_b else None
    if act != ACT_NONE:
        if want_b and plain:
            gy, gb = _K().act_bwd_bias(gz, z, act, out=tgt)
            return gy, (None if tgt is not None else gb)
        gy = _ActBwd.apply(gz, z, act)
        return gy, (_ChannelSum.apply(gy) if want_b else None)
    if want_b and tgt is not None:
        _K().channel_sum(gz, out=tgt)
        return gz, None
    return gz, (_ChannelSum.apply(gz) if want_b else None)


class _ConvBiasAct(Function):

    @staticmethod
    def forward(ctx, x, w, bias, kind, alpha, act, in_act=ACT_NONE, input_normed=False):
        ctx.kind, ctx.alpha, ctx.act, ctx.has_bias = kind, alpha, act, bias is not None
        ctx.wref, ctx.bref = w, bias
        ctx.in_act = in_act
        ctx.input_normed = bool(input_normed)
        ctx._gs_act_out = act
        ctx._gs_premasked = None
        z = kind.fwd_bias_act(x, w, bias, alpha, act)
        _tap(z, act)
        ctx.save_for_backward(x, w, z)
        return z

    @staticmethod
    def backward(ctx, gz):
        x, w, z = ctx.saved_tensors
        want_w = ctx.needs_input_grad[1] and _want_params()
        want_b = ctx.has_bias and ctx.needs_input_grad[2] and _want_params()
        act = ACT_NONE if _take_premasked(ctx, gz) else ctx.act

        def data_grad(gy):
            if not ctx.needs_input_grad[0]:
                return None
            if _PARAMS_ONLY and x.grad_fn is None and not torch.is_grad_enabled():
                return None
            if _FUSE_NORM_BWD and ctx.input_normed and not torch.is_grad_enabled() and hasattr(ctx.kind, "bwd_data_pnbwd"):
                pn = x.grad_fn
                if (isinstance(pn, _ConvBiasActNorm._backward_cls) and pn.act in (ACT_NONE, ACT_LRELU)
                        and ctx.kind.bwd_data_pnbwd_is_fused(tuple(x.shape), gy.shape[1], gy.dtype)):
                    z_prev = pn.saved_tensors[2]
                    gz_prev = _GZ.pop(z_prev.data_ptr(), None)
                    gx_ = ctx.kind.bwd_data_pnbwd(gy, w, tuple(x.shape), ctx.alpha, z_prev, pn.eps, pn.act, gz_prev)
                    if _CHECK_FUSION:
                        _check_fused("bwd_data_pnbwd", gx_, _K().pixel_norm_bwd(ctx.kind.bwd_data(gy, w, tuple(x.shape), ctx.alpha), z_prev, pn.eps, act=pn.act, addend=gz_prev))
                    pn._gs_fused = (gx_.data_ptr(), gz_prev is not None)
                    return gx_
            prod = _premask_producer(x, ctx.in_act, differentiable=True) if hasattr(ctx.kind, "bwd_data_mask") else None
            if prod is None:
                return _BilinearBwdData.apply(gy, w, x.shape, ctx.kind, ctx.alpha)
            if torch.is_grad_enabled():
                gx_ = _BwdDataMasked.apply(gy, w, x, ctx.kind, ctx.alpha, ctx.in_act)
            else:
                gx_ = ctx.kind.bwd_data_mask(gy, w, x.shape, ctx.alpha, x, ctx.in_act)
            prod._gs_premasked = gx_.data_ptr()
            return gx_

        if want_b and want_w and getattr(ctx.kind, "bias_in_wgrad", False):
            tw, tb = _accum_target(ctx.wref), _accum_target(ctx.bref)
            if tw is not None and tb is not None:
                gy = _ActBwd.apply(gz, z, act) if act != ACT_NONE else gz
                gx = data_grad(gy)
                ctx.kind.bwd_weight(x, gy, ctx.alpha, out=tw, bias_out=tb)
                return gx, None, None, None, None, None, None, None
        gy, gb = _bias_act_backward(gz, z if act != ACT_NONE else None, act, ctx.bref if want_b else None, want_b)
        gx = data_grad(gy)
        gw = None
        if want_w:
            tgt = _accum_target(ctx.wref)
            if tgt is not None:
                ctx.kind.bwd_weight(x, gy, ctx.alpha, out=tgt)
            else:
                gw = _BilinearBwdWeight.apply(x, gy, ctx.kind, ctx.alpha).to(w.dtype)
        return gx, gw, gb, None, None, None, None, None


class _PnActBwd(Function):

    @staticmethod
    def forward(ctx, g, z, eps, act):
        if act != ACT_LRELU:
            raise NotImplementedError("_PnActBwd: piecewise-linear activations only (the tanh head has no pixel norm)")
        ctx.eps, ctx.act = eps, act
        ctx._gs_done = None
        ctx.save_for_backward(g, z)
        return _K().pixel_norm_bwd(g, z, eps, act=act)

    @staticmethod
    @once_differentiable
    def backward(ctx, gg):
        g, z = ctx.saved_tensors
        done, ctx._gs_done = ctx._gs_done, None
        if ctx.needs_input_grad[0] and ctx.needs_input_grad[1]:
            if done is not None and gg.data_ptr() != done[0]:
                _handoff_broken("second-order norm gradients in the forward-on-cotangent conv")
            if done is not None:
                g_g, g_z = gg, done[1]
            else:
                g_z, g_g = _K().pixel_norm_bwd_bwd(gg, g, z, ctx.eps, pre_act=ctx.act, with_g=True)
            if _FUSE_NORM_BWD:
                _GZ[z.data_ptr()] = g_z
            return g_g, g_z, None, None
        if done is not None:
            _handoff_broken("second-order norm gradients in the forward-on-cotangent conv")
        g_g = _K().pixel_norm_bwd(gg, z, ctx.eps, pre_act=ctx.act) if ctx.needs_input_grad[0] else None
        g_z = _K().pixel_norm_bwd_bwd(gg, g, z, ctx.eps, pre_act=ctx.act) if ctx.needs_input_grad[1] else None
        return g_g, g_z, None, None


_FUSE_NORM_EPILOGUE = not config.flag("GS_NO_NORM_EPILOGUE")
_FUSE_NORM_BWD = not config.flag("GS_NO_NORM_BWD_EPILOGUE")
_FUSE_NORM_BWD2 = not config.flag("GS_NO_NORM_BWD2_EPILOGUE")

_GZ = {}


def reset_fusion_state():
    _GZ.clear()


def _handoff_broken(what):
    raise RuntimeError("gansynth_amd.functional: fused hand-off '%s' was prepared but the node received another tensor -- the single-consumer "
                       "promise of the wiring (networks.py: input_normed / input_activation, functional: sole_consumer) does not hold" % what)


_CHECK_FUSION = config.flag("GS_CHECK_FUSION")


def _check_fused(what, got, ref):
    if torch.cuda.is_available() and torch.cuda.is_current_stream_capturing():
        return
    for g, r in zip(got if isinstance(got, (tuple, list)) else (got,), ref if isinstance(ref, (tuple, list)) else (ref,)):
        scale = float(r.float().abs().max()) + 1e-30
        err = float((g.float() - r.float()).abs().max()) / scale
        tol = 1e-4 if g.dtype == torch.float32 else 4e-2
        if not err <= tol:
            raise RuntimeError("GS_CHECK_FUSION: %s differs from its unfused definition by %.3e of the tensor's scale" % (what, err))

_NORM_BWD_BIAS = not config.flag("GS_NO_NORM_BWD_BIAS")


class _ConvBiasActNorm(Function):

    @staticmethod
    def forward(ctx, x, w, bias, kind, alpha, act, eps, input_normed=False):
        ctx.kind, ctx.alpha, ctx.act, ctx.eps, ctx.has_bias = kind, alpha, act, eps, bias is not None
        ctx.wref, ctx.bref = w, bias
        ctx.input_normed = bool(input_normed)
        ctx._gs_fused = None
        ctx.set_materialize_grads(False)
        keep = any(ctx.needs_input_grad)
        want_z = keep or activation_tap.active is not None
        if _FUSE_NORM_EPILOGUE:
            z, y = kind.fwd_bias_act_norm(x, w, bias, alpha, act, eps, want_z)
        else:
            z = kind.fwd_bias_act(x, w, bias, alpha, act)
            y = _K().pixel_norm_fwd(z, eps)
        if want_z:
            _tap(z, act)
        if keep:
            ctx.save_for_backward(x, w, z)
        return y, z

    @staticmethod
    def backward(ctx, g_y, g_z):
        x, w, z = ctx.saved_tensors
        want_w = ctx.needs_input_grad[1] and _want_params()
        want_b = ctx.has_bias and ctx.needs_input_grad[2] and _want_params()
        if torch.is_grad_enabled():
            gy = _PnActBwd.apply(g_y, z, ctx.eps, ctx.act) if g_y is not None else None
            if g_z is not None:
                extra = _ActBwd.apply(g_z, z, ctx.act)
                gy = extra if gy is None else gy + extra
            sole = g_y is not None and g_z is None and not want_w and not want_b
            gx = _BilinearBwdData.apply(gy, w, x.shape, ctx.kind, ctx.alpha, sole) if ctx.needs_input_grad[0] else None
            gw = _BilinearBwdWeight.apply(x, gy, ctx.kind, ctx.alpha).to(w.dtype) if want_w else None
            gb = _ChannelSum.apply(gy) if want_b else None
            return gx, gw, gb, None, None, None, None, None
        tw = _accum_target(ctx.wref) if want_w else None
        tb = _accum_target(ctx.bref) if want_b else None
        bias_done = False
        fused, ctx._gs_fused = ctx._gs_fused, None
        if fused is not None and (g_y is None or g_y.data_ptr() != fused[0]):
            _handoff_broken("previous block's norm backward in the data-gradient conv")
        if fused is not None:
            gy = g_y
            if g_z is not None and not fused[1]:
                gy = _K().axpby(gy, _K().act_bwd(g_z, z, ctx.act), 1.0, 1.0)
        elif g_y is None:
            gy = _K().act_bwd(g_z, z, ctx.act)
        elif (tb is not None and not getattr(ctx.kind, "bias_in_wgrad", False) and _NORM_BWD_BIAS and getattr(_K(), "norm_bwd_sums_bias", False)
              and _K().norm_bwd_bias_ok(z.shape[1], z.dtype)):
            gy = _K().pixel_norm_bwd(g_y, z, ctx.eps, act=ctx.act, addend=g_z, bias_out=tb)
            bias_done = True
        else:
            gy = _K().pixel_norm_bwd(g_y, z, ctx.eps, act=ctx.act, addend=g_z)
        gx = None
        if ctx.needs_input_grad[0]:
            prod = x.grad_fn if (_FUSE_NORM_BWD and ctx.input_normed and hasattr(ctx.kind, "bwd_data_pnbwd")) else None
            if (prod is not None and isinstance(prod, _ConvBiasActNorm._backward_cls) and prod.act in (ACT_NONE, ACT_LRELU)
                    and ctx.kind.bwd_data_pnbwd_is_fused(tuple(x.shape), gy.shape[1], gy.dtype)):
                z_prev = prod.saved_tensors[2]
                gz_prev = _GZ.pop(z_prev.data_ptr(), None)
                gx = ctx.kind.bwd_data_pnbwd(gy, w, tuple(x.shape), ctx.alpha, z_prev, prod.eps, prod.act, gz_prev)
                if _CHECK_FUSION:
                    _check_fused("bwd_data_pnbwd", gx, _K().pixel_norm_bwd(ctx.kind.bwd_data(gy, w, tuple(x.shape), ctx.alpha), z_prev, prod.eps, act=prod.act, addend=gz_prev))
                prod._gs_fused = (gx.data_ptr(), gz_prev is not None)
            else:
                gx = _BilinearBwdData.apply(gy, w, x.shape, ctx.kind, ctx.alpha)
        gw = gb = None
        if bias_done:
            want_b = False
        if tw is not None and tb is not None and getattr(ctx.kind, "bias_in_wgrad", False):
            ctx.kind.bwd_weight(x, gy, ctx.alpha, out=tw, bias_out=tb)
            return gx, None, None, None, None, None, None, None
        if want_b:
            if tb is not None:
                _K().channel_sum(gy, out=tb)
            else:
                gb = _K().channel_sum(gy)
        if want_w:
            if tw is not None:
                ctx.kind.bwd_weight(x, gy, ctx.alpha, out=tw)
            else:
                gw = ctx.kind.bwd_weight(x, gy, ctx.alpha).to(w.dtype)
        return gx, gw, gb, None, None, None, None, None


def conv2d_bias_act_norm(x, w, bias, ksize, stride, alpha, act, eps, input_normed=False):
    return _ConvBiasActNorm.apply(x, w, bias, _kind(("conv", ksize, stride)), alpha, act, eps, input_normed)[0]


def conv2d_transpose_bias_act_norm(x, w, bias, alpha, act, eps, input_normed=False):
    return _ConvBiasActNorm.apply(x, w, bias, _kind(("convT",)), alpha, act, eps, input_normed)[0]


def conv2d(x, w, ksize, stride, alpha):
    return _Bilinear.apply(x, w, _kind(("conv", ksize, stride)), alpha)


def conv2d_bias_act(x, w, bias, ksize, stride, alpha, act, in_act=ACT_NONE, input_normed=False):
    return _ConvBiasAct.apply(x, w, bias, _kind(("conv", ksize, stride)), alpha, act, in_act, input_normed)


def conv2d_transpose_bias_act(x, w, bias, alpha, act):
    return _ConvBiasAct.apply(x, w, bias, _kind(("convT",)), alpha, act, ACT_NONE)


def conv2d_transpose(x, w, alpha):
    return _Bilinear.apply(x, w, _kind(("convT",)), alpha)


def dense(x, w, alpha):
    return _Bilinear.apply(x, w, _kind(("dense",)), alpha)


def dense_bias_act(x, w, bias, alpha, act):
    K = _K()
    if x.dim() == 4:
        if hasattr(K, "dense_nhwc_ok") and K.dense_nhwc_ok(x, w.shape[1]):
            return _ConvBiasAct.apply(x, w, bias, _kind(("dense_flat",)), alpha, act)
        x = x.reshape(x.shape[0], -1)
    return _ConvBiasAct.apply(x, w, bias, _kind(("dense",)), alpha, act)


def dense_of_flattened(x, w, alpha):
    K = _K()
    if hasattr(K, "dense_nhwc_ok") and x.dim() == 4 and K.dense_nhwc_ok(x, w.shape[1]):
        return _Bilinear.apply(x, w, _kind(("dense_flat",)), alpha)
    return dense(x.reshape(x.shape[0], -1), w, alpha)


class _Embedding(Function):
    @staticmethod
    def forward(ctx, idx, w, alpha, dtype):
        ctx.alpha, ctx.rows = alpha, w.shape[0]
        ctx.save_for_backward(idx)
        return _K().embedding_fwd(idx, w, alpha, dtype)

    @staticmethod
    def backward(ctx, gy):
        (idx,) = ctx.saved_tensors
        return None, (_EmbeddingBwd.apply(idx, gy, ctx.rows, ctx.alpha) if _want_params() else None), None, None


class _EmbeddingBwd(Function):
    @staticmethod
    def forward(ctx, idx, gy, rows, alpha):
        ctx.alpha, ctx.dtype = alpha, gy.dtype
        ctx.save_for_backward(idx)
        return _K().embedding_bwd(idx, gy, rows, alpha)

    @staticmethod
    def backward(ctx, ggw):
        (idx,) = ctx.saved_tensors
# ... 564 lines not shown
```

### gansynth_amd/kernels.py

```python
import contextlib
import ctypes
import os

import numpy as np
import torch

from . import config
from . import _lib
from ._lib import GS_BF16, GS_F32

CL = torch.channels_last


def _dt(t):
    if t.dtype == torch.float32:
        return GS_F32
    if t.dtype == torch.bfloat16:
        return GS_BF16
    raise TypeError(f"unsupported activation dtype {t.dtype}")


def _act(x):
    if x.dim() == 4:
        return x if x.is_contiguous(memory_format=CL) else x.contiguous(memory_format=CL)
# ... 357 lines not shown
        return y

    def conv2d_fwd_bias_act(self, x, w, bias, ksize, stride, alpha, act, bits=None):
        x, w = _act(x), _f32c(w)
        n, ci, h, wd = x.shape
        co = w.shape[3]
        bits = _bits_wanted(x, co, act) and bits is not False
        y = (_empty_act_with_bits if bits else _empty_like_act)((n, co, h // stride, wd // stride), x)
        nb = self.lib.gs_conv2d_workspace_bytes(_lib.CONV_FWD, n, h, wd, ci, co, ksize, stride, _dt(x))
        ws, prepared = self._weight_ws(w, ("fwd", ksize, stride, _dt(x)), nb, (_lib.PREP_CONV_FWD, ci, co, ksize, stride, _dt(x)))
        bp = None
        if bias is not None:
            bias = _f32c(bias)
            bp = bias.data_ptr()
        _lib.check(self.lib.gs_conv2d_fwd_bias_act(x.data_ptr(), w.data_ptr(), bp, y.data_ptr(), n, h, wd, ci, co, ksize, stride,
                                                   float(alpha), act | (_lib.ACT_WRITE_BITS if bits else 0), _dt(x), prepared, ws.data_ptr(), ws.numel(), _stream()),
                   "gs_conv2d_fwd_bias_act")
        return y

    def conv2d_fwd_bias_act_norm(self, x, w, bias, ksize, stride, alpha, act, eps, want_z=True):
        x, w = _act(x), _f32c(w)
        n, ci, h, wd = x.shape
        co = w.shape[3]
        y = _empty_like_act((n, co, h // stride, wd // stride), x)
        z = _empty_like_act((n, co, h // stride, wd // stride), x) if want_z else None
        nb = self.lib.gs_conv2d_workspace_bytes(_lib.CONV_FWD, n, h, wd, ci, co, ksize, stride, _dt(x))
        ws, prepared = self._weight_ws(w, ("fwd", ksize, stride, _dt(x)), nb, (_lib.PREP_CONV_FWD, ci, co, ksize, stride, _dt(x)))
        bp = None
        if bias is not None:
            bias = _f32c(bias)
            bp = bias.data_ptr()
        _lib.check(self.lib.gs_conv2d_fwd_bias_act_norm(x.data_ptr(), w.data_ptr(), bp, None if z is None else z.data_ptr(), y.data_ptr(), n, h, wd,
                                                        ci, co, ksize, stride, float(alpha), act, float(eps), _dt(x), prepared, ws.data_ptr(),
                                                        ws.numel(), _stream()), "gs_conv2d_fwd_bias_act_norm")
        return z, y

    def conv2d_transpose_fwd_bias_act_norm(self, x, w, bias, alpha, act, eps, want_z=True):
        x, w = _act(x), _f32c(w)
        n, ci, h, wd = x.shape
        co = w.shape[3]
        y = _empty_like_act((n, co, 2 * h, 2 * wd), x)
        z = _empty_like_act((n, co, 2 * h, 2 * wd), x) if want_z else None
        nb = self.lib.gs_conv2d_transpose_s2_workspace_bytes(_lib.CONV_FWD, n, h, wd, ci, co, _dt(x))
        ws, prepared = self._weight_ws(w, ("t_fwd", _dt(x)), nb, (_lib.PREP_CONVT_FWD, ci, co, 3, 2, _dt(x)))
        bp = None
        if bias is not None:
            bias = _f32c(bias)
            bp = bias.data_ptr()
        _lib.check(self.lib.gs_conv2d_transpose_s2_fwd_bias_act_norm(x.data_ptr(), w.data_ptr(), bp, None if z is None else z.data_ptr(), y.data_ptr(),
                                                                     n, h, wd, ci, co, float(alpha), act, float(eps), _dt(x), prepared,
                                                                     ws.data_ptr(), ws.numel(), _stream()), "gs_conv2d_transpose_s2_fwd_bias_act_norm")
        return z, y

    def conv2d_bwd_data(self, gy, w, x_shape, ksize, stride, alpha, mask=None, mask_act=0):
        gy, w = _act(gy), _f32c(w)
        n, ci, h, wd = x_shape
        co = w.shape[3]
        gx = _empty_like_act((n, ci, h, wd), gy)
        nb = self.lib.gs_conv2d_workspace_bytes(_lib.CONV_BWD_DATA, n, h, wd, ci, co, ksize, stride, _dt(gy))
        ws, prepared = self._weight_ws(w, ("bwd_data", ksize, stride, _dt(gy)), nb, (_lib.PREP_CONV_BWD_DATA, ci, co, ksize, stride, _dt(gy)))
        mp = None
        if mask is not None:
            mask = _act(mask)
            assert mask.shape == gx.shape and mask.dtype == gx.dtype
            mp = mask.data_ptr()
        _lib.check(self.lib.gs_conv2d_bwd_data_mask(gy.data_ptr(), w.data_ptr(), mp, _mask_act(mask, mask_act) if mask is not None else 0, gx.data_ptr(), n, h, wd, ci, co, ksize, stride,
                                                    float(alpha), _dt(gy), prepared, ws.data_ptr(), ws.numel(), _stream()), "gs_conv2d_bwd_data_mask")
        return gx

    def fwd_pnbwdbwd_is_fused(self, x_shape, co, ksize, stride, transposed, dtype):
        n, ci, h, wd = x_shape
        return bool(self.lib.gs_conv2d_fwd_pnbwdbwd_is_fused(int(n), int(h), int(wd), int(ci), int(co), int(ksize), int(stride), 1 if transposed else 0,
                                                            GS_F32 if dtype == torch.float32 else GS_BF16))

    def conv2d_fwd_pnbwdbwd(self, x, w, ksize, stride, alpha, g, z, eps, act):
        x, w, g, z = _act(x), _f32c(w), _act(g), _act(z)
        n, ci, h, wd = x.shape
        co = w.shape[3]
        out_g = _empty_like_act((n, co, h // stride, wd // stride), x)
        assert g.shape == out_g.shape == z.shape and g.dtype == x.dtype == z.dtype
        out_z = torch.empty_like(out_g)
        nb = self.lib.gs_conv2d_workspace_bytes(_lib.CONV_FWD, n, h, wd, ci, co, ksize, stride, _dt(x))
        ws, prepared = self._weight_ws(w, ("fwd", ksize, stride, _dt(x)), nb, (_lib.PREP_CONV_FWD, ci, co, ksize, stride, _dt(x)))
        _lib.check(self.lib.gs_conv2d_fwd_pnbwdbwd(x.data_ptr(), w.data_ptr(), g.data_ptr(), z.data_ptr(), int(act), float(eps), out_g.data_ptr(), out_z.data_ptr(), n, h,
                                                   wd, ci, co, ksize, stride, float(alpha), _dt(x), prepared, ws.data_ptr(), ws.numel(), _stream()), "gs_conv2d_fwd_pnbwdbwd")
        return out_z, out_g

    def conv2d_transpose_fwd_pnbwdbwd(self, x, w, alpha, g, z, eps, act):
        x, w, g, z = _act(x), _f32c(w), _act(g), _act(z)
        n, ci, h, wd = x.shape
        co = w.shape[3]
        out_g = _empty_like_act((n, co, 2 * h, 2 * wd), x)
        assert g.shape == out_g.shape == z.shape and g.dtype == x.dtype == z.dtype
        out_z = torch.empty_like(out_g)
        nb = self.lib.gs_conv2d_transpose_s2_workspace_bytes(_lib.CONV_FWD, n, h, wd, ci, co, _dt(x))
        ws, prepared = self._weight_ws(w, ("t_fwd", _dt(x)), nb, (_lib.PREP_CONVT_FWD, ci, co, 3, 2, _dt(x)))
        _lib.check(self.lib.gs_conv2d_transpose_s2_fwd_pnbwdbwd(x.data_ptr(), w.data_ptr(), g.data_ptr(), z.data_ptr(), int(act), float(eps), out_g.data_ptr(),
                                                                out_z.data_ptr(), n, h, wd, ci, co, float(alpha), _dt(x), prepared, ws.data_ptr(), ws.numel(), _stream()),
                   "gs_conv2d_transpose_s2_fwd_pnbwdbwd")
        return out_z, out_g

    def bwd_data_pnbwd_is_fused(self, x_shape, co, ksize, stride, transposed, dtype):
        n, ci, h, wd = x_shape
        return bool(self.lib.gs_conv2d_bwd_data_pnbwd_is_fused(int(n), int(h), int(wd), int(ci), int(co), int(ksize), int(stride), 1 if transposed else 0,
                                                              GS_F32 if dtype == torch.float32 else GS_BF16))

# ... 728 lines not shown
```

### gansynth_amd/networks.py

```python
import numpy as np
import torch

from . import config
from . import functional as F
from . import ops
from . import variables
from .variables import AUTO_REUSE, variable_scope


PIXEL_NORM_EPS = 1.0e-12
_FUSE_NORM = not config.flag("GS_NO_FUSED_NORM")


def _ilog2(ratio):
    ratio = np.asanyarray(ratio)
    depth = 0
    while not (ratio == 1).all():
        ratio = ratio >> 1
        depth += 1
    return depth


class PGGAN(object):

    def __init__(self, min_resolution, max_resolution, min_channels, max_channels, growing_level):
        self.min_resolution = np.asanyarray(min_resolution)
        self.max_resolution = np.asanyarray(max_resolution)
        self.min_channels = min_channels
        self.max_channels = max_channels
        self.growing_level = growing_level
        self.min_depth = 0
        self.fade_weight = None
        self.max_depth = _ilog2(self.max_resolution // self.min_resolution)

    @property
    def growing_depth(self):
        level = self.growing_level() if callable(self.growing_level) else self.growing_level
        full = np.float32((1 << (self.max_depth + 1)) - 1)
        return float(np.log2(np.float32(1.0) + full * np.float32(level)))

    def resolution(self, depth):
        return self.min_resolution << depth

    def channels(self, depth):
        return min(self.max_channels, self.min_channels << (self.max_depth - depth))

    def _block_name(self, kind, depth):
        return "{}_block_{}x{}".format(kind, *self.resolution(depth))

    def _head_depth(self, growing_depth):
        depth = self.min_depth
        while depth < self.max_depth and growing_depth > depth:
            depth += 1
        if depth == self.min_depth and not growing_depth > depth:
            return depth, None
        if depth == self.max_depth and growing_depth > depth:
            return depth, None
        return depth, depth - growing_depth

    def _g_conv_block(self, x, depth, sole_consumer=True):
        c = self.channels(depth)
        with variable_scope(self._block_name("conv", depth)):
            if depth == self.min_depth:
                x = ops.pixel_normalization(x)
                with variable_scope("dense"):
                    x = ops.dense_reshaped(x, c, self.resolution(depth), use_bias=True, variance_scale=2.0, scale_weight=True, activation="leaky_relu")
                    x = ops.pixel_normalization(x)
            else:
                with variable_scope("upscale_conv"):
                    x = ops.conv2d_transpose(x, filters=c, kernel_size=[3, 3], strides=[2, 2], use_bias=True,
                                             variance_scale=2.0, scale_weight=True, activation="leaky_relu",
                                             pixel_norm_epsilon=PIXEL_NORM_EPS if _FUSE_NORM else None,
                                             input_normed=sole_consumer)
                    if not _FUSE_NORM:
                        x = ops.pixel_normalization(x)
            with variable_scope("conv"):
                x = ops.conv2d(x, filters=c, kernel_size=[3, 3], use_bias=True, variance_scale=2.0, scale_weight=True,
                               activation="leaky_relu", pixel_norm_epsilon=PIXEL_NORM_EPS if _FUSE_NORM else None,
                               input_normed=depth != self.min_depth)
                if not _FUSE_NORM:
                    x = ops.pixel_normalization(x)
        return x

    def _g_color_block(self, x, depth, sole_consumer=False):
        with variable_scope(self._block_name("color", depth)):
            with variable_scope("conv"):
                return ops.conv2d(x, filters=2, kernel_size=[1, 1], use_bias=True, variance_scale=1.0, scale_weight=True,
                                  activation="tanh", input_normed=sole_consumer and _FUSE_NORM)

    def _g_variables(self, latent_dim, num_labels):
        ops.get_weight([num_labels, latent_dim], 1.0, True)
        for depth in range(self.min_depth, self.max_depth + 1):
            c = self.channels(depth)
            with variable_scope(self._block_name("conv", depth)):
                if depth == self.min_depth:
                    with variable_scope("dense"):
                        units = c * int(self.resolution(depth).prod())
                        ops.get_weight([2 * latent_dim, units], 2.0, True)
                        ops.get_bias([units])
                else:
                    with variable_scope("upscale_conv"):
                        ops.get_weight([3, 3, self.channels(depth - 1), c], 2.0, True)
                        ops.get_bias([c])
                with variable_scope("conv"):
                    ops.get_weight([3, 3, c, c], 2.0, True)
                    ops.get_bias([c])
            with variable_scope(self._block_name("color", depth)):
                with variable_scope("conv"):
                    ops.get_weight([1, 1, c, 2], 1.0, True)
                    ops.get_bias([2])

    def generator(self, latents, labels, name="generator", reuse=AUTO_REUSE):
        F.tap_begin("generator")
        with variable_scope(name, reuse=reuse):
            self._g_variables(latents.shape[1], labels.shape[1])
            embedded = ops.embedding(labels, units=latents.shape[1], variance_scale=1.0, scale_weight=True)
            x = torch.cat([latents, embedded], dim=1)
            head, fade = self._head_depth(self.growing_depth)
            for depth in range(self.min_depth, head):
                x = self._g_conv_block(x, depth)
            full = self.resolution(self.max_depth)
            middle = ops.upscale2d(self._g_color_block(self._g_conv_block(x, head, sole_consumer=fade is None), head, sole_consumer=True), full // self.resolution(head))
            if fade is None:
                return middle
            low = ops.upscale2d(self._g_color_block(x, head - 1), full // self.resolution(head - 1))
            return ops.lerp(low, middle, fade if self.fade_weight is None else self.fade_weight)

    def _d_conv_block(self, x, depth, num_labels, fresh_activation=False, sub_batches=1):
        c = self.channels(depth)
        with variable_scope(self._block_name("conv", depth)):
            if depth == self.min_depth:
                x, stddev = ops.batch_stddev_tap(x, sub_batches=sub_batches)
                with variable_scope("conv"):
                    weight, alpha = ops.get_weight([3, 3, c + 1, c], 2.0, True)
                    bias = ops.get_bias([c])
                    y = F.axpby(F.conv2d(x, F.weight_slice(weight, 0, c), 3, 1, alpha),
                                F.conv2d(stddev, F.weight_slice(weight, c, c + 1), 3, 1, alpha), 1.0, 1.0)
                    x = F.bias_act(y, bias, ops._ACT["leaky_relu"])
                with variable_scope("dense"):
                    features = ops.dense(x, units=self.channels(depth - 1), use_bias=True, variance_scale=2.0,
                                         scale_weight=True, activation="leaky_relu")
                with variable_scope("logits"):
                    logits = ops.dense(features, units=num_labels, use_bias=True, variance_scale=1.0, scale_weight=True)
                return features, logits
            with variable_scope("conv"):
                x = ops.conv2d(x, filters=c, kernel_size=[3, 3], use_bias=True, variance_scale=2.0, scale_weight=True,
                               activation="leaky_relu", input_activation="leaky_relu" if fresh_activation else None)
            with variable_scope("conv_downscale"):
                x = ops.conv2d(x, filters=self.channels(depth - 1), kernel_size=[3, 3], strides=[2, 2], use_bias=True,
                               variance_scale=2.0, scale_weight=True, activation="leaky_relu", input_activation="leaky_relu")
            return x

    def _d_color_block(self, x, depth):
        with variable_scope(self._block_name("color", depth)):
            with variable_scope("conv"):
                return ops.conv2d(x, filters=self.channels(depth), kernel_size=[1, 1], use_bias=True, variance_scale=2.0,
                                  scale_weight=True, activation="leaky_relu")

    def _d_variables(self, num_labels):
        for depth in range(self.min_depth, self.max_depth + 1):
            c = self.channels(depth)
            with variable_scope(self._block_name("color", depth)):
                with variable_scope("conv"):
                    ops.get_weight([1, 1, 2, c], 2.0, True)
                    ops.get_bias([c])
            with variable_scope(self._block_name("conv", depth)):
                if depth == self.min_depth:
                    with variable_scope("conv"):
                        ops.get_weight([3, 3, c + 1, c], 2.0, True)
                        ops.get_bias([c])
                    with variable_scope("dense"):
                        ops.get_weight([c * int(self.resolution(depth).prod()), self.channels(depth - 1)], 2.0, True)
                        ops.get_bias([self.channels(depth - 1)])
                    with variable_scope("logits"):
                        ops.get_weight([self.channels(depth - 1), num_labels], 1.0, True)
# ... 199 lines not shown
```

### gansynth_amd/ops.py

```python
import numpy as np
import torch

from . import functional as F
from . import variables
from ._lib import ACT_LRELU, ACT_NONE, ACT_TANH

_ACT = {None: ACT_NONE, "leaky_relu": ACT_LRELU, "tanh": ACT_TANH}


def _no_weight_normalizers(apply_weight_standardization, apply_spectral_normalization):
    if apply_weight_standardization:
        raise NotImplementedError("apply_weight_standardization=True (ops.py:5-25) is not on the GANSynth hot path: networks.py never sets it")
    if apply_spectral_normalization:
        raise NotImplementedError("apply_spectral_normalization=True (ops.py:28-146) is not on the GANSynth hot path: networks.py never sets it")


def get_weight(shape, variance_scale=2.0, scale_weight=False, apply_weight_standardization=False, apply_spectral_normalization=False):
    _no_weight_normalizers(apply_weight_standardization, apply_spectral_normalization)
    stddev = float(np.sqrt(variance_scale / np.prod(shape[:-1])))
    store = variables.default_store()
    if scale_weight:
        return store.get_variable("weight", shape, variables.truncated_normal(0.0, 1.0)), stddev
    return store.get_variable("weight", shape, variables.truncated_normal(0.0, stddev)), 1.0


def get_bias(shape):
    return variables.default_store().get_variable("bias", shape, variables.zeros())


def dense(inputs, units, use_bias=True, variance_scale=2.0, scale_weight=False, apply_weight_standardization=False,
          apply_spectral_normalization=False, activation=None):
    _no_weight_normalizers(apply_weight_standardization, apply_spectral_normalization)
    if inputs.dim() == 4:
        weight, alpha = get_weight([inputs.shape[1] * inputs.shape[2] * inputs.shape[3], units], variance_scale, scale_weight)
    else:
        weight, alpha = get_weight([inputs.shape[1], units], variance_scale, scale_weight)
    bias = get_bias([units]) if use_bias else None
    if bias is not None or activation is not None:
        return F.dense_bias_act(inputs, weight, bias, alpha, _ACT[activation])
    return F.dense_of_flattened(inputs, weight, alpha) if inputs.dim() == 4 else F.dense(inputs, weight, alpha)


def dense_reshaped(inputs, channels, resolution, use_bias=True, variance_scale=2.0, scale_weight=False, activation=None):
    h, w = int(resolution[0]), int(resolution[1])
    units = int(channels) * h * w
    if not F.units_nhwc_ok():
        x = dense(inputs, units=units, use_bias=use_bias, variance_scale=variance_scale, scale_weight=scale_weight)
        x = x.reshape(-1, int(channels), h, w)
        return F.bias_act(x, None, _ACT[activation]) if activation is not None else x
    weight, alpha = get_weight([inputs.shape[1], units], variance_scale, scale_weight)
    outputs = F.dense(inputs, weight, alpha)
    bias = get_bias([units]) if use_bias else None
    return F.units_bias_act_nhwc(outputs, bias, channels, h, w, _ACT[activation])


def embedding(inputs, units, variance_scale=2.0, scale_weight=False, apply_weight_standardization=False, apply_spectral_normalization=False):
    _no_weight_normalizers(apply_weight_standardization, apply_spectral_normalization)
    weight, alpha = get_weight([inputs.shape[1], units], variance_scale, scale_weight)
    return F.embedding_onehot(inputs, weight, alpha)


def conv2d(inputs, filters, kernel_size, strides=[1, 1], use_bias=True, variance_scale=2.0, scale_weight=False,
           apply_weight_standardization=False, apply_spectral_normalization=False,
           activation=None, input_activation=None, pixel_norm_epsilon=None, input_normed=False):
    _no_weight_normalizers(apply_weight_standardization, apply_spectral_normalization)
    kernel_size, strides = list(kernel_size), list(strides)
    if kernel_size[0] != kernel_size[1] or strides[0] != strides[1]:
        raise ValueError("conv2d: only square kernels / isotropic strides are on the hot path")
    weight, alpha = get_weight([*kernel_size, inputs.shape[1], filters], variance_scale, scale_weight)
    bias = get_bias([filters]) if use_bias else None
    if pixel_norm_epsilon is not None:
        return F.conv2d_bias_act_norm(inputs, weight, bias, kernel_size[0], strides[0], alpha, _ACT[activation], pixel_norm_epsilon, input_normed)
    if bias is not None or activation is not None:
        return F.conv2d_bias_act(inputs, weight, bias, kernel_size[0], strides[0], alpha, _ACT[activation], _ACT[input_activation], input_normed)
    return F.conv2d(inputs, weight, kernel_size[0], strides[0], alpha)


def conv2d_transpose(inputs, filters, kernel_size, strides=[1, 1], use_bias=True, variance_scale=2.0, scale_weight=False,
                     apply_weight_standardization=False, apply_spectral_normalization=False,
                     activation=None, pixel_norm_epsilon=None, input_normed=False):
    _no_weight_normalizers(apply_weight_standardization, apply_spectral_normalization)
    if list(kernel_size) != [3, 3] or list(strides) != [2, 2]:
        raise ValueError("conv2d_transpose: the hot path is kernel 3x3, strides 2x2 (networks.py:71-79)")
    weight, alpha = get_weight([*kernel_size, inputs.shape[1], filters], variance_scale, scale_weight)
    bias = get_bias([filters]) if use_bias else None
    if pixel_norm_epsilon is not None:
        return F.conv2d_transpose_bias_act_norm(inputs, weight, bias, alpha, _ACT[activation], pixel_norm_epsilon, input_normed)
    if bias is not None or activation is not None:
        return F.conv2d_transpose_bias_act(inputs, weight, bias, alpha, _ACT[activation])
    return F.conv2d_transpose(inputs, weight, alpha)


def upscale2d(inputs, factors=[2, 2]):
    factors = np.asanyarray(factors)
    if (factors == 1).all():
        return inputs
    return F.upscale(inputs, int(factors[0]), int(factors[1]))


def downscale2d(inputs, factors=[2, 2]):
    factors = np.asanyarray(factors)
    if (factors == 1).all():
        return inputs
    return F.avg_pool(inputs, int(factors[0]), int(factors[1]))


def pixel_normalization(inputs, epsilon=1.0e-12, input_activation=None):
    return F.pixel_norm(inputs, epsilon, _ACT[input_activation])


def batch_stddev(inputs, groups=4, epsilon=1.0e-12):
    if groups != 4:
        raise ValueError("batch_stddev: the reference graph uses groups=4 (networks.py:174)")
    if inputs.shape[0] % groups:
        raise ValueError(f"batch_stddev: batch {inputs.shape[0]} is not a multiple of groups={groups} (ops.py:341)")
    return F.batch_stddev(inputs, epsilon)


def batch_stddev_tap(inputs, groups=4, epsilon=1.0e-12, sub_batches=1):
    if groups != 4:
        raise ValueError("batch_stddev: the reference graph uses groups=4 (networks.py:174)")
    if inputs.shape[0] % (groups * sub_batches):
        raise ValueError(f"batch_stddev: batch {inputs.shape[0]} / {sub_batches} is not a multiple of groups={groups} (ops.py:341)")
    if sub_batches == 1 and not hasattr(F, "batch_stddev_tap"):
        return inputs, F.batch_stddev(inputs, epsilon)
    return F.batch_stddev_tap(inputs, epsilon, sub_batches)

# ... 42 lines not shown
```

### include/gansynth_hip.h

```cpp
#ifndef GANSYNTH_HIP_H
#define GANSYNTH_HIP_H

#include <stddef.h>
#include <stdint.h>

#ifdef __cplusplus
extern "C" {
#endif

enum { GS_F32 = 0, GS_BF16 = 1 };
enum { GS_OK = 0, GS_ERR_ARG = -1, GS_ERR_HIP = -2, GS_ERR_UNSUPPORTED = -3, GS_ERR_WORKSPACE = -4 };
enum { GS_ACT_NONE = 0, GS_ACT_LRELU = 1, GS_ACT_TANH = 2 };
enum { GS_ACT_LRELU_BITS = 5, GS_ACT_WRITE_BITS = 16 };
enum { GS_CONV_FWD = 0, GS_CONV_BWD_DATA = 1, GS_CONV_BWD_WEIGHT = 2 };

const char* gs_last_error(void);
int gs_version(void);
int gs_init(void);
int gs_streams_create(int n, void** streams);
int gs_streams_destroy(int n, void** streams);

int gs_prof_enable(int on);
int gs_prof_collect(int* launches, double* total_ms, double* total_flops);
int gs_prof_roofline(double peak_tflops, double peak_gbps, double* total_bytes, double* roof_ms, double* roof_ms_hbm_bound);
int gs_prof_records(int max_records, int* n, double* ms, double* flops, double* bytes, int* desc);

#define GS_COMM_ID_BYTES 128
typedef struct gs_comm gs_comm;
int gs_comm_available(void);
int gs_comm_unique_id(void* id128);
int gs_comm_init(gs_comm** out, int rank, int world, const void* id128);
int gs_comm_destroy(gs_comm* comm);
int gs_comm_count(gs_comm* comm, int* ranks);
int gs_allreduce_sum_f32(gs_comm* comm, float* data, int64_t count, void* stream);
int gs_comm_set_marker_us(gs_comm* comm, double us);
int gs_broadcast_f32(gs_comm* comm, float* data, int64_t count, int root, void* stream);

size_t gs_conv2d_workspace_bytes(int which, int n, int h, int w, int ci, int co, int ksize, int stride, int dtype);
int gs_conv2d_fwd(const void* x, const float* w_hwio, void* y, int n, int h, int w, int ci, int co,
                  int ksize, int stride, float alpha, int dtype, int w_prepared, void* ws, size_t ws_bytes, void* stream);
int gs_conv2d_fwd_bias_act(const void* x, const float* w_hwio, const float* bias, void* y, int n, int h, int w, int ci, int co,
                           int ksize, int stride, float alpha, int act, int dtype, int w_prepared, void* ws, size_t ws_bytes,
                           void* stream);
int gs_conv2d_bwd_data(const void* gy, const float* w_hwio, void* gx, int n, int h, int w, int ci, int co,
                       int ksize, int stride, float alpha, int dtype, int w_prepared, void* ws, size_t ws_bytes, void* stream);
int gs_conv2d_fwd_bias_act_norm(const void* x, const float* w_hwio, const float* bias, void* z, void* y, int n, int h, int w, int ci, int co,
                                int ksize, int stride, float alpha, int act, float eps, int dtype, int w_prepared, void* ws,
                                size_t ws_bytes, void* stream);
int gs_conv2d_transpose_s2_fwd_bias_act_norm(const void* x, const float* w_hwio, const float* bias, void* z, void* y, int n, int h, int w,
                                             int ci, int co, float alpha, int act, float eps, int dtype, int w_prepared, void* ws,
                                             size_t ws_bytes, void* stream);
int gs_conv2d_bwd_data_mask(const void* gy, const float* w_hwio, const void* mask, int mask_act, void* gx, int n, int h, int w, int ci, int co,
                            int ksize, int stride, float alpha, int dtype, int w_prepared, void* ws, size_t ws_bytes, void* stream);
int gs_pack_act_bits(void* z, int64_t p, int c, int dtype, void* stream);
int gs_conv2d_fwd_mask(const void* x, const float* w_hwio, const void* mask, int mask_act, void* y, int n, int h, int w, int ci, int co,
                       int ksize, int stride, float alpha, int dtype, int w_prepared, void* ws, size_t ws_bytes, void* stream);
int gs_conv2d_bwd_weight(const void* x, const void* gy, float* gw_hwio, int n, int h, int w, int ci, int co,
                         int ksize, int stride, float alpha, int accumulate, int dtype, void* ws, size_t ws_bytes, void* stream);
int gs_conv2d_bwd_weight_bias(const void* x, const void* gy, float* gw_hwio, float* gb, int n, int h, int w, int ci, int co,
                              int ksize, int stride, float alpha, int accumulate, int dtype, void* ws, size_t ws_bytes, void* stream);

size_t gs_conv2d_transpose_s2_workspace_bytes(int which, int n, int h, int w, int ci, int co, int dtype);
int gs_conv2d_transpose_s2_fwd(const void* x, const float* w_hwio, void* y, int n, int h, int w, int ci, int co,
                               float alpha, int dtype, int w_prepared, void* ws, size_t ws_bytes, void* stream);
int gs_conv2d_transpose_s2_fwd_bias_act(const void* x, const float* w_hwio, const float* bias, void* y, int n, int h, int w,
                                        int ci, int co, float alpha, int act, int dtype, int w_prepared, void* ws,
                                        size_t ws_bytes, void* stream);
int gs_conv2d_transpose_s2_bwd_data(const void* gy, const float* w_hwio, void* gx, int n, int h, int w, int ci, int co,
                                    float alpha, int dtype, int w_prepared, void* ws, size_t ws_bytes, void* stream);
int gs_conv2d_fwd_pnbwdbwd(const void* x, const float* w_hwio, const void* g, const void* z, int act, float eps, void* out_g, void* out_z, int n, int h, int w,
                           int ci, int co, int ksize, int stride, float alpha, int dtype, int w_prepared, void* ws, size_t ws_bytes, void* stream);
int gs_conv2d_transpose_s2_fwd_pnbwdbwd(const void* x, const float* w_hwio, const void* g, const void* z, int act, float eps, void* out_g, void* out_z, int n,
                                        int h, int w, int ci, int co, float alpha, int dtype, int w_prepared, void* ws, size_t ws_bytes, void* stream);
int gs_conv2d_fwd_pnbwdbwd_is_fused(int n, int h, int w, int ci, int co, int ksize, int stride, int transposed, int dtype);
int gs_conv2d_bwd_data_pnbwd(const void* gy, const float* w_hwio, const void* z, const void* addend, int act, float eps, void* gx, int n, int h, int w,
                             int ci, int co, int ksize, int stride, float alpha, int dtype, int w_prepared, void* ws, size_t ws_bytes, void* stream);
int gs_conv2d_bwd_data_pnbwd_is_fused(int n, int h, int w, int ci, int co, int ksize, int stride, int transposed, int dtype);
int gs_conv_igemm_config(int mode, int n, int hb, int wb, int ic, int oc, int dtype, int want, int* out_cfg);
int gs_conv2d_transpose_s2_bwd_data_pnbwd(const void* gy, const float* w_hwio, const void* z, const void* addend, int act, float eps, void* gx, int n,
                                          int h, int w, int ci, int co, float alpha, int dtype, int w_prepared, void* ws, size_t ws_bytes, void* stream);
int gs_conv2d_transpose_s2_bwd_weight(const void* x, const void* gy, float* gw_hwio, int n, int h, int w, int ci, int co,
                                      float alpha, int accumulate, int dtype, void* ws, size_t ws_bytes, void* stream);

typedef struct GsWgradReduce {
    const float* partials;
    float* gw;
    float* gb;
    int32_t nslices, taps, ic, oc;
    float alpha;
    int32_t transpose, accumulate;
    int32_t ic_ld;
} GsWgradReduce;
int gs_conv2d_bwd_weight_bias_partial(const void* x, const void* gy, float* gw_hwio, float* gb, int n, int h, int w, int ci, int co,
                                      int ksize, int stride, float alpha, int accumulate, int dtype, void* ws, size_t ws_bytes,
                                      GsWgradReduce* pending, void* stream);
int gs_conv2d_transpose_s2_bwd_weight_partial(const void* x, const void* gy, float* gw_hwio, int n, int h, int w, int ci, int co,
                                              float alpha, int accumulate, int dtype, void* ws, size_t ws_bytes,
                                              GsWgradReduce* pending, void* stream);
int gs_wgrad_reduce_batch(const GsWgradReduce* pending, int n, void* stream);
#define GS_WGRAD_MAX_SOURCES 4
int gs_conv2d_bwd_weight_bias_multi(const void* const* xs, const void* const* gys, const int* ns, int nsrc, unsigned bias_mask, float* gw_hwio,
                                    float* gb, int n, int h, int w, int ci, int co, int ksize, int stride, float alpha, int accumulate,
                                    int dtype, void* ws, size_t ws_bytes, GsWgradReduce* pending, void* stream);
int gs_conv2d_transpose_s2_bwd_weight_multi(const void* const* xs, const void* const* gys, const int* ns, int nsrc, float* gw_hwio, int n, int h,
// ... 142 lines not shown
```

Before: 1678 images/sec.

## Fuse generator's 1x1 colour head into the last conv's pixel-norm epilogue

Adds a colour-head epilogue to the fused conv+bias+act+pixel-norm igemm kernel for 32-channel outputs. It computes the 1x1 conv to two channels plus tanh from the normalized registers and writes the rgb output directly. The separate colour conv launch is dropped, along with its re-read of the 32-channel activation, and the normalized activation store can be skipped when nothing else needs it. The cost is extra LDS, a cross-lane reduction in the epilogue, new kernel instantiation paths and Python plumbing, and the activation is still needed for backward.

```diff
diff --git a/gansynth_amd/_lib.py b/gansynth_amd/_lib.py
--- a/gansynth_amd/_lib.py
+++ b/gansynth_amd/_lib.py
@@ -37,6 +37,9 @@
     "gs_conv2d_bwd_data": (I, [P, P, P, I, I, I, I, I, I, I, F, I, I, P, Z, P]),
     "gs_conv2d_fwd_bias_act_norm": (I, [P, P, P, P, P, I, I, I, I, I, I, I, F, I, F, I, I, P, Z, P]),
     "gs_conv2d_transpose_s2_fwd_bias_act_norm": (I, [P, P, P, P, P, I, I, I, I, I, F, I, F, I, I, P, Z, P]),
+    "gs_conv2d_fwd_rgb_is_fused": (I, [I, I, I, I, I, I, I, I, I]),
+    "gs_conv2d_fwd_bias_act_norm_rgb": (I, [P, P, P, P, P, P, P, P, F, I, I, I, I, I, I, I, F, I, F, I, I, P, Z, P]),
+    "gs_conv2d_transpose_s2_fwd_bias_act_norm_rgb": (I, [P, P, P, P, P, P, P, P, F, I, I, I, I, I, F, I, F, I, I, P, Z, P]),
     "gs_conv2d_fwd_mask": (I, [P, P, P, I, P, I, I, I, I, I, I, I, F, I, I, P, Z, P]),
     "gs_conv2d_bwd_data_mask": (I, [P, P, P, I, P, I, I, I, I, I, I, I, F, I, I, P, Z, P]),
     "gs_conv2d_bwd_weight": (I, [P, P, P, I, I, I, I, I, I, I, F, I, I, P, Z, P]),
diff --git a/gansynth_amd/config.py b/gansynth_amd/config.py
--- a/gansynth_amd/config.py
+++ b/gansynth_amd/config.py
@@ -40,6 +40,7 @@
     "GS_NO_NORM_BWD_EPILOGUE": ("ablation", "no previous-block norm backward in data-gradient epilogues"),
     "GS_NO_NORM_BWD2_EPILOGUE": ("ablation", "no second-order norm kernel in the forward-on-cotangent conv"),
     "GS_NO_NORM_BWD_BIAS": ("ablation", "bias sums outside the norm's backward"),
+    "GS_NO_COLOUR_HEAD": ("ablation", "the head block's colour conv as its own launch instead of the last conv's epilogue"),
     "GS_NO_MASK_BITS": ("ablation", "leaky-relu masks read as the bf16 activations themselves, not as the sign bits stored behind them"),
     "GS_NO_PREMASK": ("ablation", "activation derivative never folded into the consuming data-gradient kernel"),
     "GS_NO_PREMASK_GRAPH": ("ablation", "... not across autograd nodes"),
diff --git a/gansynth_amd/csrc/conv_api.hip b/gansynth_amd/csrc/conv_api.hip
--- a/gansynth_amd/csrc/conv_api.hip
+++ b/gansynth_amd/csrc/conv_api.hip
@@ -15,7 +15,7 @@
 int run_igemm(int mode, int variant, const void* x, const float* w_hwio, void* y, int N, int Hi, int Wi, int ICk,
               int OCk, int w_ci, int w_co, int Hb, int Wb, float alpha, const float* bias, int act, int dtype, int w_prepared,
               void* ws, size_t ws_bytes, hipStream_t st, const void* mask = nullptr, int mask_act = 0, void* y2 = nullptr, float pn_eps = 0.f,
-              const void* addend = nullptr, int normbwd = 0);
+              const void* addend = nullptr, int normbwd = 0, const ColourHead* head = nullptr);
 extern "C" int gs_pixel_norm_bwd_fused(const void* g, const void* x, const void* addend, void* gx, int64_t p, int c, float eps, int pre_act, int post_act, int dtype,
                                        void* stream);
 size_t wgrad_mfma_bytes(int mode, int dtype, int N, int Hb, int Wb, int IC, int OC);
@@ -895,6 +895,29 @@
     return conv2d_fwd_impl(x, w_hwio, bias, act, z, n, h, w, ci, co, ksize, stride, alpha, dtype, w_prepared, ws, ws_bytes, stream, y, eps);
 }
 
+static int check_rgb_args(const void* rgb, const float* w_rgb, int co, int act) {
+    GS_CHECK_ARG(rgb != nullptr && w_rgb != nullptr, "conv2d_fwd_bias_act_norm_rgb: rgb and its weights are required");
+    GS_CHECK_ARG(co == 32, "conv2d_fwd_bias_act_norm_rgb: the colour head rides on 32 channels (got %d)", co);
+    GS_CHECK_ARG(act == GS_ACT_NONE || act == GS_ACT_LRELU, "conv2d_fwd_bias_act_norm_rgb: activation none or leaky relu (got %d)", act);
+    return 0;
+}
+extern "C" int gs_conv2d_fwd_rgb_is_fused(int n, int h, int w, int ci, int co, int ksize, int stride, int transposed, int dtype) {
+    if (ksize != 3 || co != 32 || !igemm_supported(ci, co, dtype)) return 0;
+    if (transposed) return stride == 2 && igemm_norm_fused(MODE_T2, n, h, w, ci, co, dtype, IGEMM_NORM_FWD) ? 1 : 0;
+    return stride == 1 && igemm_norm_fused(MODE_S1, n, h, w, ci, co, dtype, IGEMM_NORM_FWD) ? 1 : 0;
+}
+extern "C" int gs_conv2d_fwd_bias_act_norm_rgb(const void* x, const float* w_hwio, const float* bias, void* z, void* y, void* rgb, const float* w_rgb,
+                                               const float* b_rgb, float rgb_alpha, int n, int h, int w, int ci, int co, int ksize, int stride, float alpha,
+                                               int act, float eps, int dtype, int w_prepared, void* ws, size_t ws_bytes, void* stream) {
+    if (int e = check_conv_args(n, h, w, ci, co, ksize, stride, dtype)) return e;
+    if (int e = check_rgb_args(rgb, w_rgb, co, act)) return e;
+    if (!gs_conv2d_fwd_rgb_is_fused(n, h, w, ci, co, ksize, stride, 0, dtype))
+        return fail(GS_ERR_UNSUPPORTED, "conv2d_fwd_bias_act_norm_rgb: no fused pixel norm for %d x %d x %d, %d -> %d channels", n, h, w, ci, co);
+    const ColourHead head = {w_rgb, b_rgb, rgb_alpha, rgb};
+    return run_igemm(MODE_S1, 0, x, w_hwio, z, n, h, w, ci, co, ci, co, h, w, alpha, bias, act, dtype, w_prepared, ws, ws_bytes, as_stream(stream), nullptr, 0, y, eps,
+                     nullptr, 0, &head);
+}
+
 extern "C" int gs_act_bwd(const void* g, const void* y, void* gx, int64_t numel, int act, int dtype, void* stream);
 
 extern "C" int gs_conv2d_bwd_data_mask(const void* gy, const float* w_hwio, const void* mask, int mask_act, void* gx, int n, int h, int w, int ci, int co,
@@ -1198,6 +1221,18 @@
     return conv2d_transpose_fwd_impl(x, w_hwio, bias, act, z, n, h, w, ci, co, alpha, dtype, w_prepared, ws, ws_bytes, stream, y, eps);
 }
 
+extern "C" int gs_conv2d_transpose_s2_fwd_bias_act_norm_rgb(const void* x, const float* w_hwio, const float* bias, void* z, void* y, void* rgb, const float* w_rgb,
+                                                            const float* b_rgb, float rgb_alpha, int n, int h, int w, int ci, int co, float alpha, int act,
+                                                            float eps, int dtype, int w_prepared, void* ws, size_t ws_bytes, void* stream) {
+    if (int e = check_conv_args(n, 2 * h, 2 * w, co, ci, 3, 2, dtype)) return e;
+    if (int e = check_rgb_args(rgb, w_rgb, co, act)) return e;
+    if (!gs_conv2d_fwd_rgb_is_fused(n, h, w, ci, co, 3, 2, 1, dtype))
+        return fail(GS_ERR_UNSUPPORTED, "conv2d_transpose_s2_fwd_bias_act_norm_rgb: no fused pixel norm for %d x %d x %d, %d -> %d channels", n, h, w, ci, co);
+    const ColourHead head = {w_rgb, b_rgb, rgb_alpha, rgb};
+    return run_igemm(MODE_T2, 0, x, w_hwio, z, n, h, w, ci, co, ci, co, h, w, alpha, bias, act, dtype, w_prepared, ws, ws_bytes, as_stream(stream), nullptr, 0, y, eps,
+                     nullptr, 0, &head);
+}
+
 extern "C" int gs_conv2d_transpose_s2_fwd_bias_act(const void* x, const float* w_hwio, const float* bias, void* y, int n, int h, int w, int ci,
                                                    int co, float alpha, int act, int dtype, int w_prepared, void* ws, size_t ws_bytes,
                                                    void* stream) {
diff --git a/gansynth_amd/csrc/conv_igemm.hip b/gansynth_amd/csrc/conv_igemm.hip
--- a/gansynth_amd/csrc/conv_igemm.hip
+++ b/gansynth_amd/csrc/conv_igemm.hip
@@ -71,6 +71,10 @@
     int N, Hi, Wi, IC, OC, Hb, Wb, tiles_x, tiles_y, nsp, noct, nch;
     unsigned m_noct, m_tx, m_ty;
     float alpha;
+    const float* head_w;
+    const float* head_b;
+    void* rgb;
+    float head_alpha;
 #ifdef GS_IGEMM_TRACE
     unsigned long long* trace;
 #endif
@@ -183,6 +187,8 @@
     unsigned char* const lpatch = lds;
     unsigned char* const lwgt = lds + NPB * PBUF;
     float* const lbias = reinterpret_cast<float*>(lwgt + (RESIDENT ? p.nch : NWB) * WBUF);
+    constexpr bool HEAD = NORM == 1 && A == 1;
+    float* const lhead = lbias + ((p.OC + 3) & ~3);
     const unsigned a_patch = (unsigned)(uintptr_t)lds;
     const unsigned a_wgt = a_patch + NPB * PBUF;
 
@@ -354,6 +360,9 @@
     }
     GS_TR(2);
     for (int c = tid; c < OC; c += (SPEC ? 512 : 256)) lbias[c] = p.bias ? p.bias[c] : 0.f;
+    if constexpr (HEAD) {
+        if (p.rgb && tid < 64) lhead[(tid & 1) * 32 + (tid >> 1)] = p.head_w[tid] * p.head_alpha;
+    }
     zero_acc();
     if (computer) {
 #pragma unroll
@@ -829,7 +838,35 @@
                                     }
 #pragma unroll
                                     for (int k = 0; k < 16; ++k) o[a][k >> 2][k & 3] *= r;
-                                    store(reinterpret_cast<T*>(p.y2), off, a, o[a], inside, static_cast<const mvec_t*>(nullptr));
+                                    if constexpr (HEAD) {
+                                        if (p.rgb) {
+                                            float d0 = 0.f, d1 = 0.f;
+#pragma unroll
+                                            for (int qd = 0; qd < 4; ++qd) {
+                                                const float4 w0 = *reinterpret_cast<const float4*>(lhead + qd * 8 + hi * 4);
+                                                const float4 w1 = *reinterpret_cast<const float4*>(lhead + 32 + qd * 8 + hi * 4);
+                                                float yv[4];
+                                                if constexpr (SZ == 4) {
+                                                    yv[0] = o[a][qd][0]; yv[1] = o[a][qd][1]; yv[2] = o[a][qd][2]; yv[3] = o[a][qd][3];
+                                                } else {
+                                                    const unsigned p01 = pack_bf16x2(o[a][qd][0], o[a][qd][1]), p23 = pack_bf16x2(o[a][qd][2], o[a][qd][3]);
+                                                    yv[0] = __uint_as_float(p01 << 16); yv[1] = __uint_as_float(p01 & 0xffff0000u);
+                                                    yv[2] = __uint_as_float(p23 << 16); yv[3] = __uint_as_float(p23 & 0xffff0000u);
+                                                }
+                                                d0 += yv[0] * w0.x; d0 += yv[1] * w0.y; d0 += yv[2] * w0.z; d0 += yv[3] * w0.w;
+                                                d1 += yv[0] * w1.x; d1 += yv[1] * w1.y; d1 += yv[2] * w1.z; d1 += yv[3] * w1.w;
+                                            }
+                                            d0 = swap32_sum(d0);
+                                            d1 = swap32_sum(d1);
+                                            if (inside && hi == 0) {
+                                                const float c0 = fast_tanh(d0 + (p.head_b ? p.head_b[0] : 0.f)), c1 = fast_tanh(d1 + (p.head_b ? p.head_b[1] : 0.f));
+                                                const long px = ((long)n * Ho + oy) * Wo + ox;
+                                                if constexpr (SZ == 4) *reinterpret_cast<float2*>(reinterpret_cast<float*>(p.rgb) + 2 * px) = make_float2(c0, c1);
+                                                else *reinterpret_cast<unsigned*>(reinterpret_cast<bf16_t*>(p.rgb) + 2 * px) = pack_bf16x2(c0, c1);
+                                            }
+                                        }
+                                    }
+                                    if (!HEAD || p.y2) store(reinterpret_cast<T*>(p.y2), off, a, o[a], inside, static_cast<const mvec_t*>(nullptr));
                                 }
                             } else {
                                 mvec_t mz_one[A][NV];
@@ -1856,6 +1893,7 @@
                 q.mask_bits = reinterpret_cast<const unsigned char*>(adv(p.mask_bits, n0 * out_img / (8 * sizeof(T))));
                 q.bits_out = reinterpret_cast<unsigned char*>(const_cast<void*>(adv(p.bits_out, n0 * out_img / (8 * sizeof(T)))));
                 q.addend = adv(p.addend, n0 * out_img);
+                q.rgb = const_cast<void*>(adv(p.rgb, n0 * (out_img / p.OC) * 2));
                 int pending = 0;
                 if (p.norm_pending) q.norm_pending = &pending;
                 if (int e = launch_igemm<T, MODE, A, B, TW, TG, RESIDENT, D, NORM, RB, SPEC, BITS>(q, st)) return e;
@@ -1866,7 +1904,9 @@
         p.m_noct = magic(p.noct); p.m_tx = magic(p.tiles_x); p.m_ty = magic(p.tiles_y);
     }
     const int wbufs = RESIDENT ? p.nch : NWB;
-    const size_t lds = (size_t)NPB * PBUF + (size_t)wbufs * WBUF + (size_t)((p.OC + 3) / 4) * 16 + 0;
+    if (p.rgb && !(NORM == 1 && A == 1 && p.OC == 32))
+        return fail(GS_ERR_UNSUPPORTED, "conv igemm: the colour head needs the fused pixel norm over 32 channels (ask gs_conv2d_fwd_rgb_is_fused first)");
+    const size_t lds = (size_t)NPB * PBUF + (size_t)wbufs * WBUF + (size_t)((p.OC + 3) / 4) * 16 + (p.rgb ? 2 * 32 * sizeof(float) : 0);
     if (p.OC % OCT != 0) return fail(GS_ERR_UNSUPPORTED, "conv igemm: %d output channels with %d-wide tiles", p.OC, OCT);
     if ((size_t)p.Hi * p.Wi * p.IC * sizeof(T) >= (1ull << 31)) return fail(GS_ERR_UNSUPPORTED, "conv igemm: one image exceeds 2 GiB");
     if (lds > 160 * 1024) return fail(GS_ERR_UNSUPPORTED, "conv igemm: %zu bytes of LDS needed", lds);
@@ -1901,7 +1941,7 @@
     if (grid >= 8) grid &= ~7L;
     const double flops = 2.0 * 9.0 * (double)p.N * p.Hb * p.Wb * p.IC * p.OC;
     const double out_px = (double)p.N * p.Hb * p.Wb * (MODE == MODE_T2 ? 4 : 1);
-    const double bytes = ((double)p.N * p.Hi * p.Wi * p.IC + out_px * p.OC * (1.0 + (p.mask ? (p.mask_bits ? 1.0 / 16.0 : 1.0) : 0.0) + (p.bits_out ? 1.0 / 16.0 : 0.0) + ((NORM == 1 && p.y) ? 1.0 : 0.0) + ((NORM == 2 && p.addend) ? 1.0 : 0.0) + (NORM == 3 ? 2.0 : 0.0)) + 9.0 * p.IC * p.OC) * sizeof(T);
+    const double bytes = ((double)p.N * p.Hi * p.Wi * p.IC + out_px * p.OC * (1.0 + (p.mask ? (p.mask_bits ? 1.0 / 16.0 : 1.0) : 0.0) + (p.bits_out ? 1.0 / 16.0 : 0.0) + ((NORM == 1 && p.y && p.y2) ? 1.0 : 0.0) + (p.rgb ? (p.y || p.y2 ? 2.0 / p.OC : 2.0 / p.OC - 1.0) : 0.0) + ((NORM == 2 && p.addend) ? 1.0 : 0.0) + (NORM == 3 ? 2.0 : 0.0)) + 9.0 * p.IC * p.OC) * sizeof(T);
     const int reps = prof_reps();
     ProfScope ps(st, flops, bytes, MODE, p.N, p.Hb, p.Wb, p.IC, p.OC, p.mask ? 1 : 0, NORM ? 1 : 0, reps);
     for (int r = 0; r < reps; ++r) hipLaunchKernelGGL(kern, dim3((unsigned)grid), dim3(SPEC ? 512 : 256), lds, st, p);
@@ -2019,7 +2059,7 @@
 template <typename T, int MODE>
 static int dispatch_igemm(ConvP p, hipStream_t st) {
     constexpr int dtype = sizeof(T) == 4 ? GS_F32 : GS_BF16;
-    const int want = p.normbwd ? 1 + p.normbwd : (p.y2 ? IGEMM_NORM_FWD : IGEMM_PLAIN);
+    const int want = p.normbwd ? 1 + p.normbwd : (p.y2 || p.rgb ? IGEMM_NORM_FWD : IGEMM_PLAIN);
     IgemmCfg c = choose_igemm(MODE, dtype, p.N, p.Hb, p.Wb, p.IC, p.OC, want, num_cus(), igemm_knobs());
 #ifdef GS_FORCE_CFG
     if (MODE == GS_FORCE_MODE && dtype == GS_BF16) c = IgemmCfg{GS_FORCE_CFG};
@@ -2059,7 +2099,7 @@
 static int run_igemm_t(int mode, int variant, const void* x, const float* w_hwio, void* y, int N, int Hi, int Wi,
                        int ICk, int OCk, int w_ci, int w_co, int Hb, int Wb, float alpha, const float* bias, int act,
                        int w_prepared, void* ws, size_t ws_bytes, hipStream_t st, const void* mask, int mask_act, void* y2, float pn_eps,
-                       const void* addend, int normbwd) {
+                       const void* addend, int normbwd, const ColourHead* head) {
     const size_t need = (size_t)9 * w_ci * w_co * sizeof(T);
     if (ws_bytes < need) return fail(GS_ERR_WORKSPACE, "conv igemm: workspace %zu < %zu", ws_bytes, need);
     T* wp = reinterpret_cast<T*>(ws);
@@ -2086,6 +2126,7 @@
     int pending = 0;
     p.y2 = y2; p.pn_eps = pn_eps; p.norm_pending = &pending;
     p.addend = normbwd ? addend : nullptr; p.normbwd = normbwd;
+    if (head) { p.head_w = head->w; p.head_b = head->bias; p.head_alpha = head->alpha; p.rgb = head->rgb; }
     int rc;
     if (mode == MODE_S1) rc = dispatch_igemm<T, MODE_S1>(p, st);
     else if (mode == MODE_S2) rc = dispatch_igemm<T, MODE_S2>(p, st);
@@ -2111,9 +2152,9 @@
 
 int run_igemm(int mode, int variant, const void* x, const float* w_hwio, void* y, int N, int Hi, int Wi, int ICk,
               int OCk, int w_ci, int w_co, int Hb, int Wb, float alpha, const float* bias, int act, int dtype, int w_prepared,
-              void* ws, size_t ws_bytes, hipStream_t st, const void* mask, int mask_act, void* y2, float pn_eps, const void* addend, int normbwd) {
+              void* ws, size_t ws_bytes, hipStream_t st, const void* mask, int mask_act, void* y2, float pn_eps, const void* addend, int normbwd, const ColourHead* head) {
     GS_DISPATCH_DTYPE(dtype, return (run_igemm_t<T>(mode, variant, x, w_hwio, y, N, Hi, Wi, ICk, OCk, w_ci, w_co, Hb,
-                                                    Wb, alpha, bias, act, w_prepared, ws, ws_bytes, st, mask, mask_act, y2, pn_eps, addend, normbwd)));
+                                                    Wb, alpha, bias, act, w_prepared, ws, ws_bytes, st, mask, mask_act, y2, pn_eps, addend, normbwd, head)));
 }
 
 static int patch_dim_rt(int mode, int t) { return mode == MODE_S1 ? t + 2 : (mode == MODE_S2 ? 2 * t + 1 : t + 1); }
diff --git a/gansynth_amd/csrc/conv_shared.h b/gansynth_amd/csrc/conv_shared.h
--- a/gansynth_amd/csrc/conv_shared.h
+++ b/gansynth_amd/csrc/conv_shared.h
@@ -5,6 +5,12 @@
 
 enum { MODE_S1 = 0, MODE_S2 = 1, MODE_T2 = 2 };
 enum { IGEMM_PLAIN = 0, IGEMM_NORM_FWD = 1, IGEMM_NORM_BWD = 2, IGEMM_NORM_BWD2 = 3 };
+struct ColourHead {
+    const float* w;
+    const float* bias;
+    float alpha;
+    void* rgb;
+};
 #define GS_WGRAD_MAX_SRC 4
 
 static inline size_t align256(size_t v) { return (v + 255) & ~(size_t)255; }
diff --git a/gansynth_amd/functional.py b/gansynth_amd/functional.py
--- a/gansynth_amd/functional.py
+++ b/gansynth_amd/functional.py
@@ -111,6 +111,13 @@
         z = self.fwd_bias_act(x, w, bias, alpha, act)
         return z, K.pixel_norm_fwd(z, eps)
 
+    def fwd_rgb_is_fused(self, x_shape, co, dtype):
+        K = _K()
+        return hasattr(K, "fwd_rgb_is_fused") and K.fwd_rgb_is_fused(x_shape, co, self.ksize, self.stride, False, dtype)
+
+    def fwd_bias_act_norm_rgb(self, x, w, bias, alpha, act, eps, head, want_z, want_y):
+        return _K().conv2d_fwd_bias_act_norm_rgb(x, w, bias, self.ksize, self.stride, alpha, act, eps, head[0], head[1], head[2], want_z=want_z, want_y=want_y)
+
     def bwd_data(self, gy, w, x_shape, alpha):
         return _K().conv2d_bwd_data(gy, w, x_shape, self.ksize, self.stride, alpha)
 
@@ -151,6 +158,13 @@
             return K.conv2d_transpose_fwd_bias_act_norm(x, w, bias, alpha, act, eps, want_z=want_z)
         z = self.fwd_bias_act(x, w, bias, alpha, act)
         return z, K.pixel_norm_fwd(z, eps)
+
+    def fwd_rgb_is_fused(self, x_shape, co, dtype):
+        K = _K()
+        return hasattr(K, "fwd_rgb_is_fused") and K.fwd_rgb_is_fused(x_shape, co, 3, 2, True, dtype)
+
+    def fwd_bias_act_norm_rgb(self, x, w, bias, alpha, act, eps, head, want_z, want_y):
+        return _K().conv2d_transpose_fwd_bias_act_norm_rgb(x, w, bias, alpha, act, eps, head[0], head[1], head[2], want_z=want_z, want_y=want_y)
 
     def bwd_data(self, gy, w, x_shape, alpha):
         return _K().conv2d_transpose_bwd_data(gy, w, alpha)
@@ -477,14 +491,14 @@
 class _ConvBiasAct(Function):
 
     @staticmethod
-    def forward(ctx, x, w, bias, kind, alpha, act, in_act=ACT_NONE, input_normed=False):
+    def forward(ctx, x, w, bias, kind, alpha, act, in_act=ACT_NONE, input_normed=False, precomputed=None):
         ctx.kind, ctx.alpha, ctx.act, ctx.has_bias = kind, alpha, act, bias is not None
         ctx.wref, ctx.bref = w, bias
         ctx.in_act = in_act
         ctx.input_normed = bool(input_normed)
         ctx._gs_act_out = act
         ctx._gs_premasked = None
-        z = kind.fwd_bias_act(x, w, bias, alpha, act)
+        z = precomputed.detach() if precomputed is not None else kind.fwd_bias_act(x, w, bias, alpha, act)
         _tap(z, act)
         ctx.save_for_backward(x, w, z)
         return z
@@ -528,7 +542,7 @@
                 gy = _ActBwd.apply(gz, z, act) if act != ACT_NONE else gz
                 gx = data_grad(gy)
                 ctx.kind.bwd_weight(x, gy, ctx.alpha, out=tw, bias_out=tb)
-                return gx, None, None, None, None, None, None, None
+                return gx, None, None, None, None, None, None, None, None
         gy, gb = _bias_act_backward(gz, z if act != ACT_NONE else None, act, ctx.bref if want_b else None, want_b)
         gx = data_grad(gy)
         gw = None
@@ -538,7 +552,7 @@
                 ctx.kind.bwd_weight(x, gy, ctx.alpha, out=tgt)
             else:
                 gw = _BilinearBwdWeight.apply(x, gy, ctx.kind, ctx.alpha).to(w.dtype)
-        return gx, gw, gb, None, None, None, None, None
+        return gx, gw, gb, None, None, None, None, None, None
 
 
 class _PnActBwd(Function):
@@ -604,12 +618,13 @@
             raise RuntimeError("GS_CHECK_FUSION: %s differs from its unfused definition by %.3e of the tensor's scale" % (what, err))
 
 _NORM_BWD_BIAS = not config.flag("GS_NO_NORM_BWD_BIAS")
+_FUSE_COLOUR_HEAD = not config.flag("GS_NO_COLOUR_HEAD")
 
 
 class _ConvBiasActNorm(Function):
 
     @staticmethod
-    def forward(ctx, x, w, bias, kind, alpha, act, eps, input_normed=False):
+    def forward(ctx, x, w, bias, kind, alpha, act, eps, input_normed=False, head=None):
         ctx.kind, ctx.alpha, ctx.act, ctx.eps, ctx.has_bias = kind, alpha, act, eps, bias is not None
         ctx.wref, ctx.bref = w, bias
         ctx.input_normed = bool(input_normed)
@@ -617,7 +632,14 @@
         ctx.set_materialize_grads(False)
         keep = any(ctx.needs_input_grad)
         want_z = keep or activation_tap.active is not None
-        if _FUSE_NORM_EPILOGUE:
+        rgb = None
+        if head is not None:
+            want_y = bool(head[3]) or _CHECK_FUSION
+            z, y, rgb = kind.fwd_bias_act_norm_rgb(x, w, bias, alpha, act, eps, head, want_z, want_y)
+            if _CHECK_FUSION:
+                _check_fused("fwd_norm_rgb", rgb, _K().conv2d_fwd_bias_act(y, head[0], head[1], 1, 1, head[2], ACT_TANH))
+            ctx.mark_non_differentiable(rgb)
+        elif _FUSE_NORM_EPILOGUE:
             z, y = kind.fwd_bias_act_norm(x, w, bias, alpha, act, eps, want_z)
         else:
             z = kind.fwd_bias_act(x, w, bias, alpha, act)
@@ -626,10 +648,10 @@
             _tap(z, act)
         if keep:
             ctx.save_for_backward(x, w, z)
-        return y, z
-
-    @staticmethod
-    def backward(ctx, g_y, g_z):
+        return (y, z) if head is None else (y, z, rgb)
+
+    @staticmethod
+    def backward(ctx, g_y, g_z, g_rgb=None):
         x, w, z = ctx.saved_tensors
         want_w = ctx.needs_input_grad[1] and _want_params()
         want_b = ctx.has_bias and ctx.needs_input_grad[2] and _want_params()
@@ -642,7 +664,7 @@
             gx = _BilinearBwdData.apply(gy, w, x.shape, ctx.kind, ctx.alpha, sole) if ctx.needs_input_grad[0] else None
             gw = _BilinearBwdWeight.apply(x, gy, ctx.kind, ctx.alpha).to(w.dtype) if want_w else None
             gb = _ChannelSum.apply(gy) if want_b else None
-            return gx, gw, gb, None, None, None, None, None
+            return gx, gw, gb, None, None, None, None, None, None
         tw = _accum_target(ctx.wref) if want_w else None
         tb = _accum_target(ctx.bref) if want_b else None
         bias_done = False
@@ -679,7 +701,7 @@
             want_b = False
         if tw is not None and tb is not None and getattr(ctx.kind, "bias_in_wgrad", False):
             ctx.kind.bwd_weight(x, gy, ctx.alpha, out=tw, bias_out=tb)
-            return gx, None, None, None, None, None, None, None
+            return gx, None, None, None, None, None, None, None, None
         if want_b:
             if tb is not None:
                 _K().channel_sum(gy, out=tb)
@@ -690,11 +712,18 @@
                 ctx.kind.bwd_weight(x, gy, ctx.alpha, out=tw)
             else:
                 gw = ctx.kind.bwd_weight(x, gy, ctx.alpha).to(w.dtype)
-        return gx, gw, gb, None, None, None, None, None
-
-
-def conv2d_bias_act_norm(x, w, bias, ksize, stride, alpha, act, eps, input_normed=False):
-    return _ConvBiasActNorm.apply(x, w, bias, _kind(("conv", ksize, stride)), alpha, act, eps, input_normed)[0]
+        return gx, gw, gb, None, None, None, None, None, None
+
+
+def conv2d_bias_act_norm(x, w, bias, ksize, stride, alpha, act, eps, input_normed=False, colour_head=None):
+    kind = _kind(("conv", ksize, stride))
+    if colour_head is None:
+        return _ConvBiasActNorm.apply(x, w, bias, kind, alpha, act, eps, input_normed)[0]
+    if (_FUSE_COLOUR_HEAD and _FUSE_NORM_EPILOGUE and act in (ACT_NONE, ACT_LRELU) and x.dtype in (torch.float32, torch.bfloat16)
+            and kind.fwd_rgb_is_fused(tuple(x.shape), w.shape[3], x.dtype)):
+        y, _, rgb = _ConvBiasActNorm.apply(x, w, bias, kind, alpha, act, eps, input_normed, tuple(colour_head) + (torch.is_grad_enabled(),))
+        return y, rgb
+    return _ConvBiasActNorm.apply(x, w, bias, kind, alpha, act, eps, input_normed)[0], None
 
 
 def conv2d_transpose_bias_act_norm(x, w, bias, alpha, act, eps, input_normed=False):
@@ -705,8 +734,10 @@
     return _Bilinear.apply(x, w, _kind(("conv", ksize, stride)), alpha)
 
 
-def conv2d_bias_act(x, w, bias, ksize, stride, alpha, act, in_act=ACT_NONE, input_normed=False):
-    return _ConvBiasAct.apply(x, w, bias, _kind(("conv", ksize, stride)), alpha, act, in_act, input_normed)
+def conv2d_bias_act(x, w, bias, ksize, stride, alpha, act, in_act=ACT_NONE, input_normed=False, precomputed=None):
+    if precomputed is not None and x is None:
+        return precomputed
+    return _ConvBiasAct.apply(x, w, bias, _kind(("conv", ksize, stride)), alpha, act, in_act, input_normed, precomputed)
 
 
 def conv2d_transpose_bias_act(x, w, bias, alpha, act):
diff --git a/gansynth_amd/kernels.py b/gansynth_amd/kernels.py
--- a/gansynth_amd/kernels.py
+++ b/gansynth_amd/kernels.py
@@ -433,6 +433,40 @@
                                                                      ws.data_ptr(), ws.numel(), _stream()), "gs_conv2d_transpose_s2_fwd_bias_act_norm")
         return z, y
 
+    def fwd_rgb_is_fused(self, x_shape, co, ksize, stride, transposed, dtype):
+        n, ci, h, wd = x_shape
+        return bool(self.lib.gs_conv2d_fwd_rgb_is_fused(int(n), int(h), int(wd), int(ci), int(co), int(ksize), int(stride), 1 if transposed else 0,
+                                                       GS_F32 if dtype == torch.float32 else GS_BF16))
+
+    def conv2d_fwd_bias_act_norm_rgb(self, x, w, bias, ksize, stride, alpha, act, eps, w_rgb, b_rgb, rgb_alpha, want_z=True, want_y=True, transposed=False):
+        x, w, w_rgb = _act(x), _f32c(w), _f32c(w_rgb)
+        n, ci, h, wd = x.shape
+        co = w.shape[3]
+        assert tuple(w_rgb.shape) == (1, 1, co, 2), tuple(w_rgb.shape)
+        out = (n, co, 2 * h, 2 * wd) if transposed else (n, co, h // stride, wd // stride)
+        y = _empty_like_act(out, x) if want_y else None
+        z = _empty_like_act(out, x) if want_z else None
+        rgb = _empty_like_act((n, 2, out[2], out[3]), x)
+        bp = _f32c(bias) if bias is not None else None
+        brp = _f32c(b_rgb) if b_rgb is not None else None
+        ptr = lambda t: None if t is None else t.data_ptr()
+        if transposed:
+            nb = self.lib.gs_conv2d_transpose_s2_workspace_bytes(_lib.CONV_FWD, n, h, wd, ci, co, _dt(x))
+            ws, prepared = self._weight_ws(w, ("t_fwd", _dt(x)), nb, (_lib.PREP_CONVT_FWD, ci, co, 3, 2, _dt(x)))
+            _lib.check(self.lib.gs_conv2d_transpose_s2_fwd_bias_act_norm_rgb(x.data_ptr(), w.data_ptr(), ptr(bp), ptr(z), ptr(y), rgb.data_ptr(), w_rgb.data_ptr(), ptr(brp),
+                                                                             float(rgb_alpha), n, h, wd, ci, co, float(alpha), act, float(eps), _dt(x), prepared,
+                                                                             ws.data_ptr(), ws.numel(), _stream()), "gs_conv2d_transpose_s2_fwd_bias_act_norm_rgb")
+        else:
+            nb = self.lib.gs_conv2d_workspace_bytes(_lib.CONV_FWD, n, h, wd, ci, co, ksize, stride, _dt(x))
+            ws, prepared = self._weight_ws(w, ("fwd", ksize, stride, _dt(x)), nb, (_lib.PREP_CONV_FWD, ci, co, ksize, stride, _dt(x)))
+            _lib.check(self.lib.gs_conv2d_fwd_bias_act_norm_rgb(x.data_ptr(), w.data_ptr(), ptr(bp), ptr(z), ptr(y), rgb.data_ptr(), w_rgb.data_ptr(), ptr(brp), float(rgb_alpha),
+                                                                n, h, wd, ci, co, ksize, stride, float(alpha), act, float(eps), _dt(x), prepared, ws.data_ptr(),
+                                                                ws.numel(), _stream()), "gs_conv2d_fwd_bias_act_norm_rgb")
+        return z, y, rgb
+
+    def conv2d_transpose_fwd_bias_act_norm_rgb(self, x, w, bias, alpha, act, eps, w_rgb, b_rgb, rgb_alpha, want_z=True, want_y=True):
+        return self.conv2d_fwd_bias_act_norm_rgb(x, w, bias, 3, 2, alpha, act, eps, w_rgb, b_rgb, rgb_alpha, want_z=want_z, want_y=want_y, transposed=True)
+
     def conv2d_bwd_data(self, gy, w, x_shape, ksize, stride, alpha, mask=None, mask_act=0):
         gy, w = _act(gy), _f32c(w)
         n, ci, h, wd = x_shape
diff --git a/gansynth_amd/networks.py b/gansynth_amd/networks.py
--- a/gansynth_amd/networks.py
+++ b/gansynth_amd/networks.py
@@ -58,8 +58,15 @@
             return depth, None
         return depth, depth - growing_depth
 
-    def _g_conv_block(self, x, depth, sole_consumer=True):
+    def _g_color_variables(self, depth):
+        with variable_scope(self._block_name("color", depth)):
+            with variable_scope("conv"):
+                weight, alpha = ops.get_weight([1, 1, self.channels(depth), 2], 1.0, True)
+                return weight, ops.get_bias([2]), alpha
+
+    def _g_conv_block(self, x, depth, sole_consumer=True, color_head=False):
         c = self.channels(depth)
+        head = self._g_color_variables(depth) if color_head and _FUSE_NORM else None
         with variable_scope(self._block_name("conv", depth)):
             if depth == self.min_depth:
                 x = ops.pixel_normalization(x)
@@ -77,16 +84,22 @@
             with variable_scope("conv"):
                 x = ops.conv2d(x, filters=c, kernel_size=[3, 3], use_bias=True, variance_scale=2.0, scale_weight=True,
                                activation="leaky_relu", pixel_norm_epsilon=PIXEL_NORM_EPS if _FUSE_NORM else None,
-                               input_normed=depth != self.min_depth)
+                               input_normed=depth != self.min_depth,
+                               colour_head=head)
                 if not _FUSE_NORM:
                     x = ops.pixel_normalization(x)
-        return x
-
-    def _g_color_block(self, x, depth, sole_consumer=False):
+        if not color_head:
+            return x
+        if head is None:
+            return x, None
+        x, rgb = x
+        return x, (None if rgb is None else (rgb, c))
+
+    def _g_color_block(self, x, depth, sole_consumer=False, rgb=None):
         with variable_scope(self._block_name("color", depth)):
             with variable_scope("conv"):
                 return ops.conv2d(x, filters=2, kernel_size=[1, 1], use_bias=True, variance_scale=1.0, scale_weight=True,
-                                  activation="tanh", input_normed=sole_consumer and _FUSE_NORM)
+                                  activation="tanh", input_normed=sole_consumer and _FUSE_NORM, precomputed=rgb)
 
     def _g_variables(self, latent_dim, num_labels):
         ops.get_weight([num_labels, latent_dim], 1.0, True)
@@ -120,7 +133,8 @@
             for depth in range(self.min_depth, head):
                 x = self._g_conv_block(x, depth)
             full = self.resolution(self.max_depth)
-            middle = ops.upscale2d(self._g_color_block(self._g_conv_block(x, head, sole_consumer=fade is None), head, sole_consumer=True), full // self.resolution(head))
+            y, rgb = self._g_conv_block(x, head, sole_consumer=fade is None, color_head=True)
+            middle = ops.upscale2d(self._g_color_block(y, head, sole_consumer=True, rgb=rgb), full // self.resolution(head))
             if fade is None:
                 return middle
             low = ops.upscale2d(self._g_color_block(x, head - 1), full // self.resolution(head - 1))
diff --git a/gansynth_amd/ops.py b/gansynth_amd/ops.py
--- a/gansynth_amd/ops.py
+++ b/gansynth_amd/ops.py
@@ -62,17 +62,20 @@
 
 def conv2d(inputs, filters, kernel_size, strides=[1, 1], use_bias=True, variance_scale=2.0, scale_weight=False,
            apply_weight_standardization=False, apply_spectral_normalization=False,
-           activation=None, input_activation=None, pixel_norm_epsilon=None, input_normed=False):
+           activation=None, input_activation=None, pixel_norm_epsilon=None, input_normed=False, colour_head=None, precomputed=None):
     _no_weight_normalizers(apply_weight_standardization, apply_spectral_normalization)
     kernel_size, strides = list(kernel_size), list(strides)
     if kernel_size[0] != kernel_size[1] or strides[0] != strides[1]:
         raise ValueError("conv2d: only square kernels / isotropic strides are on the hot path")
-    weight, alpha = get_weight([*kernel_size, inputs.shape[1], filters], variance_scale, scale_weight)
+    in_channels = inputs.shape[1] if inputs is not None else precomputed[1]
+    weight, alpha = get_weight([*kernel_size, in_channels, filters], variance_scale, scale_weight)
     bias = get_bias([filters]) if use_bias else None
     if pixel_norm_epsilon is not None:
-        return F.conv2d_bias_act_norm(inputs, weight, bias, kernel_size[0], strides[0], alpha, _ACT[activation], pixel_norm_epsilon, input_normed)
+        return F.conv2d_bias_act_norm(inputs, weight, bias, kernel_size[0], strides[0], alpha, _ACT[activation], pixel_norm_epsilon, input_normed,
+                                      colour_head=colour_head)
     if bias is not None or activation is not None:
-        return F.conv2d_bias_act(inputs, weight, bias, kernel_size[0], strides[0], alpha, _ACT[activation], _ACT[input_activation], input_normed)
+        return F.conv2d_bias_act(inputs, weight, bias, kernel_size[0], strides[0], alpha, _ACT[activation], _ACT[input_activation], input_normed,
+                                 precomputed=None if precomputed is None else precomputed[0])
     return F.conv2d(inputs, weight, kernel_size[0], strides[0], alpha)
 
 
diff --git a/include/gansynth_hip.h b/include/gansynth_hip.h
--- a/include/gansynth_hip.h
+++ b/include/gansynth_hip.h
@@ -50,6 +50,13 @@
 int gs_conv2d_transpose_s2_fwd_bias_act_norm(const void* x, const float* w_hwio, const float* bias, void* z, void* y, int n, int h, int w,
                                              int ci, int co, float alpha, int act, float eps, int dtype, int w_prepared, void* ws,
                                              size_t ws_bytes, void* stream);
+int gs_conv2d_fwd_rgb_is_fused(int n, int h, int w, int ci, int co, int ksize, int stride, int transposed, int dtype);
+int gs_conv2d_fwd_bias_act_norm_rgb(const void* x, const float* w_hwio, const float* bias, void* z, void* y, void* rgb, const float* w_rgb,
+                                    const float* b_rgb, float rgb_alpha, int n, int h, int w, int ci, int co, int ksize, int stride, float alpha,
+                                    int act, float eps, int dtype, int w_prepared, void* ws, size_t ws_bytes, void* stream);
+int gs_conv2d_transpose_s2_fwd_bias_act_norm_rgb(const void* x, const float* w_hwio, const float* bias, void* z, void* y, void* rgb, const float* w_rgb,
+                                                 const float* b_rgb, float rgb_alpha, int n, int h, int w, int ci, int co, float alpha, int act,
+                                                 float eps, int dtype, int w_prepared, void* ws, size_t ws_bytes, void* stream);
 int gs_conv2d_bwd_data_mask(const void* gy, const float* w_hwio, const void* mask, int mask_act, void* gx, int n, int h, int w, int ci, int co,
                             int ksize, int stride, float alpha, int dtype, int w_prepared, void* ws, size_t ws_bytes, void* stream);
 int gs_pack_act_bits(void* z, int64_t p, int c, int dtype, void* stream);
```

After: 1693 images/sec (median of 6 runs). Within noise of the previous version (+0.9%).
